# BGU-CS-VIL/DPMMSubClusters.jl

Measured on NVIDIA B200. Metric: gibbs_iters_per_sec, higher is better.
Workload: dtype f32

## Files before the change

dpmmsubclusters.jl_b200/_lib.py:

```python
from __future__ import annotations

import ctypes as C
import os

_HERE = os.path.dirname(os.path.abspath(__file__))
LIB_PATH = os.environ.get("DPMM_LIB_PATH") or os.path.join(_HERE, "libdpmm_b200.so")

OK, EINVAL, ECUDA, ESTATE, ELIMIT, ENCCL = 0, -1, -2, -3, -4, -5
PRIOR_NIW, PRIOR_MULTINOMIAL = 0, 1
SAMPLER_INVERSE_CDF, SAMPLER_GUMBEL = 0, 1

_p = C.c_void_p
_i32, _i64, _u64 = C.c_int32, C.c_int64, C.c_uint64
_f32p, _f64p, _i64p, _u8p = (C.POINTER(C.c_float), C.POINTER(C.c_double), C.POINTER(C.c_int64),
                             C.POINTER(C.c_uint8))

SIGNATURES = {
    "dpmm_create": (C.c_int, [C.POINTER(_p), _f32p, _i64, _i32, _i32, _i32, _u64, _i64]),
    "dpmm_destroy": (C.c_int, [_p]),
    "dpmm_last_error": (C.c_char_p, [_p]),
    "dpmm_set_stream": (C.c_int, [_p, _p]),
    "dpmm_sync": (C.c_int, [_p]),
    "dpmm_limits": (C.c_int, [C.POINTER(_i32)]),
    "dpmm_init_labels": (C.c_int, [_p, _i32, _i32]),
    "dpmm_randomize_sublabels": (C.c_int, [_p, _i64p, _i32]),
    "dpmm_get_labels": (C.c_int, [_p, _i64p]),
    "dpmm_get_sublabels": (C.c_int, [_p, _i64p]),
    "dpmm_set_labels": (C.c_int, [_p, _i64p]),
    "dpmm_set_sublabels": (C.c_int, [_p, _i64p]),
    "dpmm_set_params_niw": (C.c_int, [_p, _i32, _f32p, _f32p, _f32p, _f32p, _f32p]),
    "dpmm_set_params_multinomial": (C.c_int, [_p, _i32, _f32p, _f32p, _f32p]),
    "dpmm_set_sampler": (C.c_int, [_p, _i32]),
    "dpmm_sample_labels": (C.c_int, [_p, _i32]),
    "dpmm_sample_sublabels": (C.c_int, [_p]),
    "dpmm_suff_stats": (C.c_int, [_p, _i64p, _i32, _i64p, _f64p, _f64p]),
    "dpmm_num_clusters": (C.c_int, [_p]),
    "dpmm_set_hyper_niw": (C.c_int, [_p, C.c_double, _f64p, C.c_double, _f64p, C.c_double]),
    "dpmm_set_hyper_multinomial": (C.c_int, [_p, _f32p, C.c_double]),
    "dpmm_posterior_step": (C.c_int, [_p, _i64p, _i32, _i32, _u8p, _i32, _i64p, _f64p, _f64p]),
    "dpmm_sample_params": (C.c_int, [_p, _i32, _i32, _i32]),
    "dpmm_params_merge": (C.c_int, [_p, _i64, _i64]),
    "dpmm_get_params_niw": (C.c_int, [_p, _i32, _f32p, _f64p, _f32p, _f32p, _f32p]),
    "dpmm_get_params_multinomial": (C.c_int, [_p, _i32, _f32p, _f32p, _f32p]),
    "dpmm_predict_niw": (C.c_int, [_p, _i32, _f32p, _f32p, _f32p, _f32p, _i64p, _f32p]),
    "dpmm_predict_multinomial": (C.c_int, [_p, _i32, _f64p, _f32p, _i64p, _f32p]),
    "dpmm_apply_split": (C.c_int, [_p, _i64p, _i64p, _i32]),
    "dpmm_apply_merge": (C.c_int, [_p, _i64p, _i64p, _i32]),
    "dpmm_remove_empty": (C.c_int, [_p, _i64p, _i32]),
    "dpmm_smart_project": (C.c_int, [_p, _i64, _f64p, _f64p, _f64p, _i64p]),
    "dpmm_smart_kmeans_iter": (C.c_int, [_p, C.c_double, C.c_double, _f64p]),
    "dpmm_smart_set_sublabels": (C.c_int, [_p, _i64]),
    "dpmm_nccl_unique_id": (C.c_int, [_p]),
    "dpmm_comm_init": (C.c_int, [_p, _p, _i32, _i32]),
    "dpmm_set_uniforms": (C.c_int, [_p, _f64p, _f64p, _u8p]),
    "dpmm_debug_loglik": (C.c_int, [_p, _i32, _f32p]),
    "dpmm_debug_tc_stats": (C.c_int, [_p, _i64p]),
    "dpmm_debug_fused_stats": (C.c_int, [_p, _i64p]),
    "dpmm_timing_enable": (C.c_int, [_p, _i32]),
    "dpmm_timing_kinds": (C.c_int, []),
    "dpmm_timing_name": (C.c_char_p, [_i32]),
    "dpmm_timing_read": (C.c_int, [_p, _f64p, _i64p, _i32]),
    "dpmm_launch_count": (_i64, [_p]),
}

_lib = None


class DpmmError(RuntimeError):
    def __init__(self, code, msg):
        super().__init__(f"libdpmm_b200 error {code}: {msg}")
        self.code = code


def load():
    global _lib
    if _lib is not None:
        return _lib
    if not os.path.exists(LIB_PATH):
        raise FileNotFoundError(
            f"{LIB_PATH} is missing: build it with `python -c 'import __graft_entry__ as g; g.build()'` "
            "(nvcc, sm_100a). This package has no CPU fallback.")
    lib = C.CDLL(LIB_PATH)
    for name, (res, args) in SIGNATURES.items():
        fn = getattr(lib, name)
        fn.restype = res
        fn.argtypes = args
    _lib = lib
    return lib


def check(rc, ctx=None):
    if rc != 0:
        msg = load().dpmm_last_error(ctx)
        raise DpmmError(rc, msg.decode() if msg else "?")
```

dpmmsubclusters.jl_b200/csrc/common.cuh:

```cuda
#pragma once
#include <cuda_runtime.h>
#include <cstdint>
#include <math_constants.h>

#include "philox.cuh"

#define DPMM_MAX_K 1024
#define DPMM_MNM_MAX_D 16384

typedef unsigned long long f32x2_t;
__device__ __forceinline__ f32x2_t f2_pack(float lo, float hi) {
  f32x2_t r;
  asm("mov.b64 %0, {%1, %2};" : "=l"(r) : "f"(lo), "f"(hi));
  return r;
}
__device__ __forceinline__ void f2_unpack(f32x2_t v, float& lo, float& hi) {
  asm("mov.b64 {%0, %1}, %2;" : "=f"(lo), "=f"(hi) : "l"(v));
}
__device__ __forceinline__ f32x2_t f2_fma(f32x2_t a, f32x2_t b, f32x2_t c) {
  f32x2_t d;
  asm("fma.rn.f32x2 %0, %1, %2, %3;" : "=l"(d) : "l"(a), "l"(b), "l"(c));
  return d;
}

// ... 106 lines not shown
    const int k = __ffsll((long long)m) - 1;
    const float e = rs[k * stride];
    const bool zero = (e < 1.17549435e-38f) && s_regular;
    const float quo = __fdiv_rn(zero ? 1.f : e, s);
    cw = __fadd_rn(cw, zero ? 0.f : quo);
    rs[k * stride] = cw;
  }
  const double t = u * (double)cw;
  if (!(0.0 < t) && !(mask & 1ull)) return 0;
  for (uint64_t m = mask; m; m &= m - 1) {
    const int k = __ffsll((long long)m) - 1;
    if (k >= K - 1) break;
    if (!((double)rs[k * stride] < t)) return k;
  }
  return K - 1;
}

__device__ __forceinline__ int dpmm_draw_inverse_cdf_screened(float* rs, int stride, int K, double u) {
  if (K > 64) return dpmm_draw_inverse_cdf(rs, stride, K, u);
  float mx = -CUDART_INF_F;
  bool has_nan = false;
  for (int k = 0; k < K; ++k) {
    const float v = rs[k * stride];
    has_nan |= (v != v);
    mx = fmaxf(mx, v);
  }
  if (has_nan || !(mx > -CUDART_INF_F) || !(mx < CUDART_INF_F)) return dpmm_draw_inverse_cdf(rs, stride, K, u);
  const float thr = mx - 104.f;
  uint64_t mask = 0;
  for (int k = 0; k < K; ++k)
    if (rs[k * stride] >= thr) mask |= 1ull << k;
  if (2 * __popcll(mask) > K) return dpmm_draw_inverse_cdf(rs, stride, K, u);
  return dpmm_draw_inverse_cdf_masked(rs, stride, K, mask, u);
}

__device__ __forceinline__ int dpmm_draw_argmax(const float* rs, int stride, int K) {
  int best = 0;
  float bv = rs[0];
  if (bv != bv) return 0;
  for (int k = 1; k < K; ++k) {
    const float v = rs[k * stride];
    if (v != v) return k;
    if (v > bv) {
      bv = v;
      best = k;
    }
  }
  return best;
}

__device__ __forceinline__ int dpmm_draw_gumbel(const float* rs, int stride, int K, uint64_t seed,
                                               uint32_t call, uint64_t gidx) {
  int best = 0;
  float bv = -CUDART_INF_F;
  for (int k0 = 0; k0 < K; k0 += 4) {
    const Philox4 r = philox4x32_10((uint32_t)gidx, (uint32_t)(gidx >> 32), call,
                                    DPMM_STREAM_GUMBEL + 8u * (uint32_t)(k0 >> 2), (uint32_t)seed,
                                    (uint32_t)(seed >> 32));
    const uint32_t w[4] = {r.x, r.y, r.z, r.w};
#pragma unroll
    for (int j = 0; j < 4; ++j) {
      const int k = k0 + j;
      if (k < K) {
        float v = rs[k * stride];
        if (v != v) v = -CUDART_INF_F;
        const float uu = ((float)w[j] + 0.5f) * 2.3283064365386963e-10f;
        const float g = -__logf(-__logf(uu));
        const float t = v + g;
        if (t > bv || k == 0) {
          bv = t;
          best = k;
        }
      }
    }
  }
  return best;
}

__device__ __forceinline__ int dpmm_draw_two(float rl, float rr, double u) {
  float m[2] = {rl, rr};
  return dpmm_draw_inverse_cdf(m, 1, 2, u);
}

__device__ __forceinline__ double dpmm_uniform(const double* inj, int64_t local_i, uint64_t seed,
                                               uint32_t stream, uint32_t call, uint64_t gidx) {
  if (inj != nullptr) return inj[local_i];
  return philox_to_uniform(philox_draw(seed, stream, call, gidx));
}

__device__ __forceinline__ int dpmm_randbit(const uint8_t* inj, int64_t local_i, uint64_t seed,
                                            uint32_t call, uint64_t gidx) {
  if (inj != nullptr) return inj[local_i] & 1;
  return (int)(philox_draw(seed, DPMM_STREAM_RANDBITS, call, gidx).x & 1u);
}
```

dpmmsubclusters.jl_b200/csrc/ctx.cuh:

```cuda
#pragma once
#include "../../include/dpmm_b200.h"

#include <cuda.h>
#include <cuda_runtime.h>

#include <algorithm>
#include <cmath>
#include <cstdio>
#include <cstdlib>
#include <cstring>
#include <string>
#include <vector>

struct StatsItem;
struct SmartState;

enum TimingKind {
  TK_LABEL = 0,
  TK_SORT,
  TK_SUBLABEL,
  TK_STATS,
  TK_STATS_AUX,
  TK_RELABEL,
  TK_ALLREDUCE,
  TK_LABEL_OVF,
  TK_PARAMS,
  TK_COUNT
};
static const char* const kTimingNames[TK_COUNT] = {"label", "sort", "sublabel", "stats", "stats_aux", "relabel", "allreduce", "label_ovf", "params"};

struct TimedEvent {
  cudaEvent_t a, b;
  int kind;
};

struct UidBlob {
  char b[128];
};
struct NcclApi {
  void* handle = nullptr;
  int (*GetUniqueId)(void*) = nullptr;
  int (*CommInitRank)(void**, int, UidBlob, int) = nullptr;
  int (*AllReduce)(const void*, void*, size_t, int, int, void*, cudaStream_t) = nullptr;
  int (*AllGather)(const void*, void*, size_t, int, void*, cudaStream_t) = nullptr;
  int (*CommDestroy)(void*) = nullptr;
  const char* (*GetErrorString)(int) = nullptr;
};
struct dpmm_ctx {
  int device = 0;
  int sm_count = 148;
  int smem_optin = 0;
  int smem_per_sm = 0;
  cudaStream_t stream = nullptr;
  bool own_stream = true;
  cudaStream_t side = nullptr;
  cudaEvent_t ev_fork = nullptr, ev_join = nullptr;
  int64_t n = 0;
  int D = 0;
  int D_user = 0;
  int prior = 0;
  uint64_t seed = 0;
  int64_t goff = 0;
  uint32_t call = 0;
  int sampler = 0;
  std::string err;

  float* x = nullptr;
  int32_t* labels = nullptr;
  uint8_t* sub = nullptr;
  int32_t* perm = nullptr;
  int32_t* perm2 = nullptr;
  int64_t* wide = nullptr;
  int32_t* wide_status = nullptr;
  double* u_label = nullptr;
  double* u_sub = nullptr;
  uint8_t* r_bits = nullptr;

  int K = 0, Kcap = 0;
  int label_bound = 1;
  bool params_set = false;
  int rec_f = 0;
  float* raw_params = nullptr;
  float* recs = nullptr;
  float* cst = nullptr;
  float* logw = nullptr;
  float* loglr = nullptr;
  float* tc_w = nullptr;
  float* tc_b = nullptr;
  float* tc_mu = nullptr;
  float* tc_fro = nullptr;
  int32_t* tc_stats = nullptr;
  float* t2_piv = nullptr;
  float* t2_scr = nullptr;
  float* t2_u = nullptr;
  float* t2_bias = nullptr;
  float* t2_fro8 = nullptr;
  int32_t* t2_ctr = nullptr;
  int32_t* ctr_sets = nullptr;
  int ctr_cur = 0;
  bool ctr_clean = false;
  bool t2_ok = false;
  bool t2_params = false;
  int t2_KS = 0, t2_nch = 0;
  int32_t* t2_hstat = nullptr;
  cudaEvent_t t2_hstat_ev = nullptr;
  bool t2_hstat_pending = false;
  int t2_cooldown = 0;
  float* ss_w = nullptr;
  float* ss_b = nullptr;
  float* ss_c = nullptr;
  int32_t* lcount = nullptr;
  CUtensorMap tmap_x;
  float* mtc_w = nullptr;
  bool mtc_ok = false;
  bool mtc_params = false;
  bool tc_ok = false;
  bool tc_params = false;
  float* logp_t = nullptr;
  int KP = 0;
  int32_t* hist = nullptr;
  int32_t* seg_off = nullptr;
  int32_t* scat_cursor = nullptr;
  int32_t* lr_cursor = nullptr;
  int32_t* lut_l = nullptr;
  int32_t* lut_r = nullptr;
  uint8_t* rule = nullptr;
  uint8_t* wanted = nullptr;
  int32_t* idx_list = nullptr;
  int stats_rec = 0;
  double* acc = nullptr;
  float* centers = nullptr;
  double* outbuf = nullptr;
  StatsItem* items = nullptr;
  int64_t items_cap = 0;
  int32_t* item_ctr = nullptr;
  int chunk = 1024;

  void* hstage = nullptr;
  size_t hstage_bytes = 0;
  void* hup[2] = {nullptr, nullptr};
  size_t hup_bytes[2] = {0, 0};
  cudaEvent_t hup_ev[2] = {nullptr, nullptr};
  int hup_i = 0;

  bool hist_valid = false, sorted = false, partitioned = false;
  bool scan_valid = false;
  int64_t n_fused = 0, n_cached = 0, n_recompute = 0;
  bool acc_cleared = false;
  bool stats_cached = false;
  bool cursors_fresh = false;
  int64_t launches = 0;
  bool timing = false;
  std::vector<TimedEvent> tev;
  std::vector<cudaEvent_t> ev_pool;
  double t_ms[TK_COUNT] = {0};
  int64_t t_n[TK_COUNT] = {0};

  bool dev_params = false;
  double alpha = 0.0;
  double* hyper_d = nullptr;
  double* ptab = nullptr;
  double* ptab_alt = nullptr;
  double* post = nullptr;
  double* post_alt = nullptr;
  double* lfac = nullptr;
  double* pm_out = nullptr;
  uint8_t* splittable_d = nullptr;
  int32_t* newof_d = nullptr;
  float* w_out = nullptr;
  float* lr_out = nullptr;
  uint32_t pcall = 0;
  int Kcap_tab = 0;

  SmartState* smart = nullptr;

  NcclApi nccl;
  void* comm = nullptr;
  int world = 1, rank = 0;
  bool ipc_ok = false;
  uint8_t* ipc_local = nullptr;
  uint8_t* ipc_peer[16] = {nullptr};
  size_t ipc_cap = 0;
  uint32_t ipc_epoch = 0;
};

void dpmm_internal_smart_free(dpmm_ctx* ctx);
int dpmm_internal_ensure_sorted(dpmm_ctx* ctx);

inline thread_local std::string g_err;

inline int fail(dpmm_ctx* c, int code, const std::string& msg) {
  if (c) c->err = msg;
  g_err = msg;
  return code;
}
#define CK(call)                                                                                   \
  do {                                                                                             \
    cudaError_t e__ = (call);                                                                      \
    if (e__ != cudaSuccess)                                                                        \
      return fail(ctx, DPMM_ECUDA, std::string(#call) + ": " + cudaGetErrorString(e__));          \
  } while (0)
#define NEED(cond, code, msg) \
  do {                        \
// ... 99 lines not shown
```

dpmmsubclusters.jl_b200/csrc/dpmm_b200.cu:

```cuda

#include <dlfcn.h>

#include <algorithm>
#include <cmath>
#include <cstdio>
#include <cstring>
#include <string>
#include <vector>

#include "common.cuh"
#include "kernels_gauss.cuh"
#include "kernels_gauss_tc.cuh"
#include "kernels_gauss_tc2.cuh"
#include "kernels_ipc.cuh"
#include "kernels_mnm.cuh"
#include "kernels_mnm_tc.cuh"
#include "kernels_pack.cuh"
#include "kernels_params.cuh"
#include "kernels_params_mnm.cuh"
#include "kernels_sort.cuh"
#include "kernels_stats.cuh"
#include "kernels_stats_tc.cuh"
#include "kernels_stats_tc64.cuh"
#include "kernels_substats_tc.cuh"
// ... 8 lines not shown
  return gauss_col_off(D) + ((D + 3) & ~3);
}

template <typename T>
static cudaError_t dev_grow_keep(T** p, size_t old_count, size_t new_count) {
  T* q = nullptr;
  cudaError_t e = cudaMalloc((void**)&q, std::max<size_t>(new_count, 1) * sizeof(T));
  if (e != cudaSuccess) return e;
  e = cudaMemset(q, 0, std::max<size_t>(new_count, 1) * sizeof(T));
  if (e == cudaSuccess && *p && old_count) e = cudaMemcpy(q, *p, old_count * sizeof(T), cudaMemcpyDeviceToDevice);
  if (*p) cudaFree(*p);
  *p = q;
  return e;
}
static int post_doubles(const dpmm_ctx* c) {
  return c->prior == DPMM_PRIOR_NIW ? NIW_POST_DOUBLES(c->D) : MNM_POST_DOUBLES(c->D);
}
static int ensure_tables(dpmm_ctx* ctx, int cap) {
  if (cap <= ctx->Kcap_tab) return 0;
  CK(cudaStreamSynchronize(ctx->stream));
  const int D = ctx->D, old = ctx->Kcap_tab;
  const bool niw = ctx->prior == DPMM_PRIOR_NIW;
  const size_t rec3 = (size_t)3 * (niw ? 1 + D + D * D : 1 + D), post3 = (size_t)3 * post_doubles(ctx);
  CK(dev_grow_keep(&ctx->ptab, old * rec3, cap * rec3));
  CK(dev_grow_keep(&ctx->ptab_alt, 0, cap * rec3));
  CK(dev_grow_keep(&ctx->post, old * post3, cap * post3));
  CK(dev_grow_keep(&ctx->post_alt, 0, cap * post3));
  if (niw) CK(dev_grow_keep(&ctx->lfac, (size_t)3 * old * D * D, (size_t)3 * cap * D * D));
  CK(dev_grow_keep(&ctx->pm_out, 0, (size_t)cap * 6 + (size_t)cap * cap + 2));
  CK(dev_grow_keep(&ctx->splittable_d, 0, (size_t)cap));
  CK(dev_grow_keep(&ctx->newof_d, 0, (size_t)cap));
  CK(dev_grow_keep(&ctx->w_out, (size_t)old, (size_t)cap));
  CK(dev_grow_keep(&ctx->lr_out, (size_t)2 * old, (size_t)2 * cap));
  ctx->Kcap_tab = cap;
  return 0;
}

static int ensure_k(dpmm_ctx* ctx, int K) {
  if (K <= ctx->Kcap) return 0;
  int cap = std::max(K, std::max(8, ctx->Kcap * 2));
  cap = std::min(cap, DPMM_MAX_K);
  if (K > cap) return fail(ctx, DPMM_ELIMIT, "K exceeds DPMM_MAX_K");
  CK(cudaStreamSynchronize(ctx->stream));
  const int D = ctx->D;
  ctx->rec_f = nrec_floats(ctx);
  ctx->stats_rec = (ctx->prior == DPMM_PRIOR_NIW) ? 1 + D + D * D : 1 + D;
  CK(dev_realloc(&ctx->recs, (size_t)3 * cap * ctx->rec_f));
  if (ctx->prior == DPMM_PRIOR_NIW) CK(dev_realloc(&ctx->raw_params, (size_t)3 * cap * (D + D * D + 1)));
  CK(dev_realloc(&ctx->cst, (size_t)3 * cap));
  CK(dev_realloc(&ctx->logw, (size_t)cap));
  CK(dev_realloc(&ctx->loglr, (size_t)2 * cap));
  if (ctx->prior == DPMM_PRIOR_MULTINOMIAL) CK(dev_realloc(&ctx->logp_t, (size_t)D * (cap + MNM_KT)));
  if (ctx->mtc_ok) {
    CK(dev_realloc(&ctx->mtc_w, (size_t)3 * ((D + 31) / 32) * MTC_N * 32));
    ctx->mtc_params = false;
  }
  if (ctx->tc_ok || ctx->t2_ok) {
    CK(dev_realloc(&ctx->tc_b, (size_t)cap * D));
    CK(dev_realloc(&ctx->tc_mu, (size_t)cap * D));
    CK(dev_realloc(&ctx->tc_fro, (size_t)cap));
    ctx->tc_params = ctx->t2_params = false;
  }
  if (ctx->t2_ok) {
    const int capt = std::min(cap, T2_MAX_K);
    CK(dev_realloc(&ctx->t2_piv, (size_t)capt * D * D));
    CK(dev_realloc(&ctx->t2_u, (size_t)capt * D * D));
    CK(dev_realloc(&ctx->t2_scr, (size_t)gauss_tc2_nch(D, capt) * (D / 8) * 1024));
    CK(dev_realloc(&ctx->t2_bias, (size_t)capt * (gauss_tc2_nch(D, capt) * 512 + 32)));
    CK(dev_realloc(&ctx->t2_fro8, (size_t)capt));
  }
  if (ctx->tc_ok) {
    const int capc = std::min(cap, TC_MAX_K);
    CK(dev_realloc(&ctx->tc_w, (size_t)((capc + TC_NCL - 1) / TC_NCL) * TC_NCL * TC_D * TC_D));
    CK(dev_realloc(&ctx->ss_w, (size_t)cap * 2 * SS_D * SS_D));
    CK(dev_realloc(&ctx->ss_b, (size_t)cap * 2 * SS_D));
    CK(dev_realloc(&ctx->ss_c, (size_t)cap * SS_D));
    CK(dev_realloc(&ctx->lcount, (size_t)cap));
  }
  if (ctx->prior == DPMM_PRIOR_NIW && D == L64_D) {
    CK(dev_realloc(&ctx->ss_w, (size_t)cap * 2 * D * D));
    CK(dev_realloc(&ctx->ss_b, (size_t)cap * 2 * D));
    CK(dev_realloc(&ctx->ss_c, (size_t)cap * D));
  }
  CK(dev_realloc(&ctx->hist, (size_t)cap));
  CK(dev_realloc(&ctx->seg_off, (size_t)cap + 1));
  CK(dev_realloc(&ctx->scat_cursor, (size_t)cap));
  CK(dev_realloc(&ctx->lr_cursor, (size_t)2 * cap));
  CK(dev_realloc(&ctx->lut_l, (size_t)cap));
  CK(dev_realloc(&ctx->lut_r, (size_t)cap));
  CK(dev_realloc(&ctx->rule, (size_t)cap));
  CK(dev_realloc(&ctx->wanted, (size_t)cap));
  CK(dev_realloc(&ctx->idx_list, (size_t)cap));
  CK(dev_realloc(&ctx->acc, (size_t)2 * cap * ctx->stats_rec));
  CK(dev_realloc(&ctx->centers, (size_t)2 * cap * ctx->D));
  CK(dev_realloc(&ctx->outbuf, (size_t)3 * cap * ctx->stats_rec + 1));
  ctx->items_cap = ctx->n / ctx->chunk + 2 * (int64_t)cap + 2;
  CK(dev_realloc(&ctx->items, (size_t)ctx->items_cap));
  ctx->Kcap = cap;
  ctx->hist_valid = ctx->scan_valid = ctx->sorted = ctx->partitioned = ctx->stats_cached = false;
  ctx->params_set = false;
  ctx->acc_cleared = ctx->cursors_fresh = false;
  if (ctx->dev_params) {
    int rc = ensure_tables(ctx, cap);
    if (rc) return rc;
  }
  return 0;
}

#define DPMM_NIW_DIMS(X) X(1) X(2) X(3) X(4) X(5) X(6) X(7) X(8) X(12) X(16) X(24) X(32) X(48) X(64)

static bool niw_dim_supported(int D) {
  switch (D) {
#define X(d) case d:
    DPMM_NIW_DIMS(X)
#undef X
    return true;
    default:
      return false;
  }
}

#define DECL_SET(n)                                                                              \
  int niw_set_label_##n(dpmm_ctx*, const GaussLabelArgs&, int, int*);                            \
  int niw_set_sublabel_##n(dpmm_ctx*, const SubLabelArgs&, bool, int, int*);                     \
  int niw_set_stats_##n(dpmm_ctx*, const StatsArgs&, int, int*);
DECL_SET(0) DECL_SET(1) DECL_SET(2) DECL_SET(3) DECL_SET(4) DECL_SET(5)
#undef DECL_SET

int niw_launch_label(dpmm_ctx* ctx, const GaussLabelArgs& a) {
  int rc = DPMM_ELIMIT;
  const int D = ctx->D;
  if (niw_set_label_0(ctx, a, D, &rc) && niw_set_label_1(ctx, a, D, &rc) && niw_set_label_2(ctx, a, D, &rc) &&
      niw_set_label_3(ctx, a, D, &rc) && niw_set_label_4(ctx, a, D, &rc) && niw_set_label_5(ctx, a, D, &rc))
    return fail(ctx, DPMM_ELIMIT, "NIW: no kernel instantiated for this D");
  return rc;
}
int niw_launch_sublabel(dpmm_ctx* ctx, const SubLabelArgs& a, bool sample) {
  int rc = DPMM_ELIMIT;
  const int D = ctx->D;
  if (niw_set_sublabel_0(ctx, a, sample, D, &rc) && niw_set_sublabel_1(ctx, a, sample, D, &rc) &&
      niw_set_sublabel_2(ctx, a, sample, D, &rc) && niw_set_sublabel_3(ctx, a, sample, D, &rc) &&
      niw_set_sublabel_4(ctx, a, sample, D, &rc) && niw_set_sublabel_5(ctx, a, sample, D, &rc))
    return fail(ctx, DPMM_ELIMIT, "NIW: no kernel instantiated for this D");
  return rc;
}
int niw_launch_stats(dpmm_ctx* ctx, const StatsArgs& a) {
  int rc = DPMM_ELIMIT;
  const int D = ctx->D;
  if (niw_set_stats_0(ctx, a, D, &rc) && niw_set_stats_1(ctx, a, D, &rc) && niw_set_stats_2(ctx, a, D, &rc) &&
      niw_set_stats_3(ctx, a, D, &rc) && niw_set_stats_4(ctx, a, D, &rc) && niw_set_stats_5(ctx, a, D, &rc))
    return fail(ctx, DPMM_ELIMIT, "NIW: no kernel instantiated for this D");
  return rc;
}

extern "C" const char* dpmm_last_error(const dpmm_ctx* ctx) { return ctx ? ctx->err.c_str() : g_err.c_str(); }

extern "C" int dpmm_limits(int32_t* out3) {
  if (!out3) return DPMM_EINVAL;
  out3[0] = 64;
  out3[1] = DPMM_MNM_MAX_D;
  out3[2] = DPMM_MAX_K;
  return 0;
}

extern "C" int dpmm_create(dpmm_ctx** out, const float* x, int64_t n_local, int32_t d, int32_t prior_kind,
                           int32_t device, uint64_t seed, int64_t global_offset) {
  dpmm_ctx* ctx = nullptr;
// ... 6 lines not shown
  if (prior_kind == DPMM_PRIOR_NIW) {
    NEED(d <= 64, DPMM_ELIMIT, "NIW: D must be <= 64");
    while (!niw_dim_supported(dpad)) ++dpad;
  } else
    NEED(d <= DPMM_MNM_MAX_D, DPMM_ELIMIT, "multinomial: D must be <= 16384");
  int ndev = 0;
  if (cudaGetDeviceCount(&ndev) != cudaSuccess || ndev == 0)
    return fail(nullptr, DPMM_ECUDA, "no CUDA device: libdpmm_b200 has no CPU fallback");
  NEED(device >= 0 && device < ndev, DPMM_EINVAL, "bad device ordinal");
  ctx = new dpmm_ctx();
  ctx->device = device;
  ctx->n = n_local;
  ctx->D = dpad;
  ctx->D_user = d;
  ctx->prior = prior_kind;
  ctx->seed = seed;
  ctx->goff = global_offset;
  auto bail = [&](int code) {
    g_err = ctx->err;
    dpmm_destroy(ctx);
    return code;
  };
#define CKC(call)                                                                        \
  do {                                                                                   \
    cudaError_t e__ = (call);                                                            \
    if (e__ != cudaSuccess) {                                                            \
      ctx->err = std::string(#call) + ": " + cudaGetErrorString(e__);                    \
      return bail(DPMM_ECUDA);                                                           \
    }                                                                                    \
  } while (0)
  CKC(cudaSetDevice(device));
  cudaDeviceProp prop;
  CKC(cudaGetDeviceProperties(&prop, device));
  if (prop.major < 10) {
    ctx->err = "device is not sm_100-class (Blackwell); this library ships sm_100a code only";
    return bail(DPMM_ECUDA);
  }
  ctx->sm_count = prop.multiProcessorCount;
  ctx->smem_optin = (int)prop.sharedMemPerBlockOptin;
  ctx->smem_per_sm = (int)prop.sharedMemPerMultiprocessor;
  CKC(cudaStreamCreateWithFlags(&ctx->stream, cudaStreamNonBlocking));
  CKC(cudaMalloc((void**)&ctx->x, (size_t)n_local * dpad * sizeof(float)));
  CKC(cudaMalloc((void**)&ctx->labels, (size_t)n_local * sizeof(int32_t)));
  CKC(cudaMalloc((void**)&ctx->sub, (size_t)n_local));
  CKC(cudaMalloc((void**)&ctx->perm, (size_t)n_local * sizeof(int32_t)));
  CKC(cudaMalloc((void**)&ctx->perm2, (size_t)n_local * sizeof(int32_t)));
  CKC(cudaMalloc((void**)&ctx->item_ctr, 2 * sizeof(int32_t)));
  if (dpad == d) {
    CKC(cudaMemcpyAsync(ctx->x, x, (size_t)n_local * d * sizeof(float), cudaMemcpyHostToDevice, ctx->stream));
  } else {
    float* raw = nullptr;
    CKC(cudaMalloc((void**)&raw, (size_t)n_local * d * sizeof(float)));
    cudaError_t e1 = cudaMemcpyAsync(raw, x, (size_t)n_local * d * sizeof(float), cudaMemcpyHostToDevice, ctx->stream);
    if (e1 == cudaSuccess) {
      pad_points_kernel<<<(unsigned)prop.multiProcessorCount * 8, 256, 0, ctx->stream>>>(raw, n_local, d, dpad, ctx->x);
      e1 = cudaGetLastError();
    }
    if (e1 == cudaSuccess) e1 = cudaStreamSynchronize(ctx->stream);
    cudaFree(raw);
    CKC(e1);
  }
  CKC(cudaMemsetAsync(ctx->labels, 0, (size_t)n_local * sizeof(int32_t), ctx->stream));
  CKC(cudaMemsetAsync(ctx->sub, 0, (size_t)n_local, ctx->stream));
  CKC(cudaStreamSynchronize(ctx->stream));
  if (prior_kind == DPMM_PRIOR_NIW && dpad == TC_D && n_local >= TC_TILE) {
    typedef CUresult (*EncodeFn)(CUtensorMap*, CUtensorMapDataType, cuuint32_t, void*, const cuuint64_t*, const cuuint64_t*,
                                 const cuuint32_t*, const cuuint32_t*, CUtensorMapInterleave, CUtensorMapSwizzle,
                                 CUtensorMapL2promotion, CUtensorMapFloatOOBfill);
    void* fn = nullptr;
    cudaDriverEntryPointQueryResult qres;
    if (cudaGetDriverEntryPoint("cuTensorMapEncodeTiled", &fn, cudaEnableDefault, &qres) == cudaSuccess && fn != nullptr &&
        qres == cudaDriverEntryPointSuccess) {
      const cuuint64_t gdim[2] = {(cuuint64_t)TC_D, (cuuint64_t)n_local};
      const cuuint64_t gstr[1] = {(cuuint64_t)TC_D * 4};
      const cuuint32_t box[2] = {TC_D, TC_TILE};
      const cuuint32_t estr[2] = {1, 1};
      const CUresult r = ((EncodeFn)fn)(&ctx->tmap_x, CU_TENSOR_MAP_DATA_TYPE_FLOAT32, 2, ctx->x, gdim, gstr, box, estr,
                                        CU_TENSOR_MAP_INTERLEAVE_NONE, CU_TENSOR_MAP_SWIZZLE_128B,
                                        CU_TENSOR_MAP_L2_PROMOTION_L2_128B, CU_TENSOR_MAP_FLOAT_OOB_FILL_NONE);
      ctx->tc_ok = (r == CUDA_SUCCESS);
    }
  }
  if (ctx->tc_ok || (prior_kind == DPMM_PRIOR_NIW && (dpad == 32 || dpad == 64) && n_local >= T2_TILE)) {
    CKC(cudaMalloc((void**)&ctx->ctr_sets, 8 * sizeof(int32_t)));
    CKC(cudaMemset(ctx->ctr_sets, 0, 8 * sizeof(int32_t)));
    ctx->tc_stats = ctx->ctr_sets;
    ctx->t2_ctr = ctx->ctr_sets + 2;
  }
  if (prior_kind == DPMM_PRIOR_NIW && (dpad == 32 || dpad == 64) && n_local >= T2_TILE) ctx->t2_ok = true;
  if (prior_kind == DPMM_PRIOR_MULTINOMIAL && d % 4 == 0 && d <= MTC_MAX_D && n_local >= MTC_TILE) {
    bool exact = false;
    {
      int32_t* flag = nullptr;
      int32_t hflag = 1;
      if (cudaMalloc((void**)&flag, 4) == cudaSuccess) {
        cudaMemsetAsync(flag, 0, 4, ctx->stream);
        tf32_exact_scan_kernel<<<(unsigned)ctx->sm_count * 16, 256, 0, ctx->stream>>>(ctx->x, (int64_t)n_local * d, flag);
        if (cudaMemcpyAsync(&hflag, flag, 4, cudaMemcpyDeviceToHost, ctx->stream) == cudaSuccess &&
            cudaStreamSynchronize(ctx->stream) == cudaSuccess)
          exact = hflag == 0;
        cudaFree(flag);
      }
    }
    typedef CUresult (*EncodeFn)(CUtensorMap*, CUtensorMapDataType, cuuint32_t, void*, const cuuint64_t*, const cuuint64_t*,
                                 const cuuint32_t*, const cuuint32_t*, CUtensorMapInterleave, CUtensorMapSwizzle,
                                 CUtensorMapL2promotion, CUtensorMapFloatOOBfill);
    void* fn = nullptr;
    cudaDriverEntryPointQueryResult qres;
    if (exact && cudaGetDriverEntryPoint("cuTensorMapEncodeTiled", &fn, cudaEnableDefault, &qres) == cudaSuccess &&
        fn != nullptr && qres == cudaDriverEntryPointSuccess) {
      const cuuint64_t gdim[2] = {(cuuint64_t)d, (cuuint64_t)n_local};
      const cuuint64_t gstr[1] = {(cuuint64_t)d * 4};
      const cuuint32_t box[2] = {32, MTC_TILE};
      const cuuint32_t estr[2] = {1, 1};
      const CUresult r = ((EncodeFn)fn)(&ctx->tmap_x, CU_TENSOR_MAP_DATA_TYPE_FLOAT32, 2, ctx->x, gdim, gstr, box, estr,
                                        CU_TENSOR_MAP_INTERLEAVE_NONE, CU_TENSOR_MAP_SWIZZLE_128B,
                                        CU_TENSOR_MAP_L2_PROMOTION_L2_128B, CU_TENSOR_MAP_FLOAT_OOB_FILL_NONE);
      ctx->mtc_ok = (r == CUDA_SUCCESS);
    }
  }
#undef CKC
  ctx->chunk = prior_kind == DPMM_PRIOR_NIW ? 1024 : 256;
  *out = ctx;
  return 0;
}

extern "C" int dpmm_destroy(dpmm_ctx* ctx) {
  if (!ctx) return 0;
  cudaSetDevice(ctx->device);
  if (ctx->stream) cudaStreamSynchronize(ctx->stream);
  if (env_int("DPMM_VERBOSE", 0))
    fprintf(stderr, "[dpmm] fused sub-label+statistics launches %lld, statistics served from them %lld, exact recomputations %lld\n",
            (long long)ctx->n_fused, (long long)ctx->n_cached, (long long)ctx->n_recompute);
  for (int p = 0; p < IPC_MAX_WORLD; ++p)
    if (ctx->ipc_peer[p]) cudaIpcCloseMemHandle(ctx->ipc_peer[p]);
  if (ctx->ipc_local) cudaFree(ctx->ipc_local);
  dpmm_internal_smart_free(ctx);
  if (ctx->side) {
    cudaStreamSynchronize(ctx->side);
    cudaStreamDestroy(ctx->side);
    cudaEventDestroy(ctx->ev_fork);
    cudaEventDestroy(ctx->ev_join);
  }
  if (ctx->comm && ctx->nccl.CommDestroy) ctx->nccl.CommDestroy(ctx->comm);
  for (auto& t : ctx->tev) {
    cudaEventDestroy(t.a);
    cudaEventDestroy(t.b);
  }
  for (auto e : ctx->ev_pool) cudaEventDestroy(e);
  void* ptrs[] = {ctx->x, ctx->labels, ctx->sub, ctx->perm, ctx->perm2, ctx->u_label, ctx->u_sub, ctx->r_bits,
                  ctx->raw_params, ctx->recs, ctx->cst, ctx->logw, ctx->loglr, ctx->logp_t, ctx->t2_piv, ctx->t2_scr, ctx->t2_u, ctx->t2_bias, ctx->t2_fro8, ctx->ctr_sets, ctx->tc_w, ctx->tc_b, ctx->tc_mu, ctx->tc_fro, ctx->ss_w, ctx->ss_b, ctx->ss_c, ctx->lcount, ctx->mtc_w, ctx->hist, ctx->seg_off,
                  ctx->scat_cursor, ctx->lr_cursor, ctx->lut_l, ctx->lut_r, ctx->rule, ctx->wanted,
                  ctx->idx_list, ctx->acc, ctx->centers, ctx->outbuf, ctx->items, ctx->item_ctr, ctx->hyper_d, ctx->ptab,
                  ctx->ptab_alt, ctx->post, ctx->post_alt, ctx->lfac, ctx->pm_out, ctx->splittable_d, ctx->newof_d,
                  ctx->w_out, ctx->lr_out, ctx->wide, ctx->wide_status};
  for (void* p : ptrs)
    if (p) cudaFree(p);
  if (ctx->hstage) cudaFreeHost(ctx->hstage);
  if (ctx->t2_hstat) cudaFreeHost(ctx->t2_hstat);
  if (ctx->t2_hstat_ev) cudaEventDestroy(ctx->t2_hstat_ev);
  for (int i = 0; i < 2; ++i) {
    if (ctx->hup[i]) cudaFreeHost(ctx->hup[i]);
    if (ctx->hup_ev[i]) cudaEventDestroy(ctx->hup_ev[i]);
  }
  if (ctx->own_stream && ctx->stream) cudaStreamDestroy(ctx->stream);
  delete ctx;
  return 0;
}

extern "C" int dpmm_set_stream(dpmm_ctx* ctx, void* cuda_stream) {
  NEED(ctx, DPMM_EINVAL, "ctx is NULL");
  CK(cudaSetDevice(ctx->device));
  CK(cudaStreamSynchronize(ctx->stream));
  if (ctx->own_stream && ctx->stream) cudaStreamDestroy(ctx->stream);
  ctx->stream = (cudaStream_t)cuda_stream;
  ctx->own_stream = false;
  return 0;
}

extern "C" int dpmm_sync(dpmm_ctx* ctx) {
  NEED(ctx, DPMM_EINVAL, "ctx is NULL");
  CK(cudaSetDevice(ctx->device));
  CK(cudaStreamSynchronize(ctx->stream));
  return 0;
}

extern "C" int dpmm_set_sampler(dpmm_ctx* ctx, int32_t sampler) {
  NEED(ctx, DPMM_EINVAL, "ctx is NULL");
  NEED(sampler == DPMM_SAMPLER_INVERSE_CDF || sampler == DPMM_SAMPLER_GUMBEL, DPMM_EINVAL, "unknown sampler");
  ctx->sampler = sampler;
  return 0;
}

static int run_relabel(dpmm_ctx* ctx, const std::vector<int32_t>& ll, const std::vector<int32_t>& lr,
                       const std::vector<uint8_t>& rule, bool uses_rng) {
  const int K = (int)ll.size();
  int rc = ensure_k(ctx, K);
  if (rc) return rc;
  const size_t b4 = (size_t)K * 4;
  void* hs = nullptr;
  const int slot = upload_acquire(ctx, 2 * b4 + K, &hs);
  if (slot < 0) return slot;
  char* h = (char*)hs;
  memcpy(h, ll.data(), b4);
  memcpy(h + b4, lr.data(), b4);
  memcpy(h + 2 * b4, rule.data(), K);
  CK(cudaMemcpyAsync(ctx->lut_l, h, b4, cudaMemcpyHostToDevice, ctx->stream));
  CK(cudaMemcpyAsync(ctx->lut_r, h + b4, b4, cudaMemcpyHostToDevice, ctx->stream));
  CK(cudaMemcpyAsync(ctx->rule, h + 2 * b4, K, cudaMemcpyHostToDevice, ctx->stream));
  rc = upload_release(ctx, slot);
  if (rc) return rc;
  if (uses_rng) ctx->call += 1;
  {
    KernelTimer kt(ctx, TK_RELABEL);
    const int T = 256;
    const unsigned grid = (unsigned)std::min<int64_t>((ctx->n + T - 1) / T, (int64_t)ctx->sm_count * 16);
    relabel_kernel<<<grid, T, 0, ctx->stream>>>(ctx->labels, ctx->sub, ctx->n, K, ctx->lut_l, ctx->lut_r, ctx->rule,
                                                ctx->r_bits, ctx->seed, ctx->call, ctx->goff);
    CK(cudaGetLastError());
  }
  return 0;
}

extern "C" int dpmm_init_labels(dpmm_ctx* ctx, int32_t init_clusters, int32_t outlier) {
  NEED(ctx, DPMM_EINVAL, "ctx is NULL");
  NEED(init_clusters >= 1 && init_clusters + (outlier ? 1 : 0) <= DPMM_MAX_K, DPMM_EINVAL, "bad init_clusters");
  CK(cudaSetDevice(ctx->device));
  ctx->label_bound = init_clusters + (outlier ? 1 : 0);
  {
    int rc = ensure_k(ctx, ctx->label_bound);
    if (rc) return rc;
  }
  ctx->call += 1;
  {
// ... 301 lines not shown
  const size_t raw_floats = nrec * D + nrec * D * D + nrec;
  const size_t bytes = (raw_floats + K + 2 * K) * sizeof(float);
  void* hs = nullptr;
  const int slot = upload_acquire(ctx, bytes, &hs);
  if (slot < 0) return slot;
  float* h_mu = (float*)hs;
  float* h_inv = h_mu + nrec * D;
  float* h_ld = h_inv + nrec * D * D;
  float* h_logw = h_ld + nrec;
  float* h_loglr = h_logw + K;
  if (Du == D) {
    memcpy(h_mu, mu, nrec * D * 4);
    memcpy(h_inv, inv_sigma, nrec * D * D * 4);
  } else {
    memset(h_mu, 0, nrec * D * 4);
    memset(h_inv, 0, nrec * D * D * 4);
    for (size_t t = 0; t < nrec; ++t) {
      memcpy(h_mu + t * D, mu + t * Du, (size_t)Du * 4);
      for (int i = 0; i < Du; ++i) memcpy(h_inv + (t * D + i) * D, inv_sigma + (t * Du + i) * Du, (size_t)Du * 4);
      for (int i = Du; i < D; ++i) h_inv[(t * D + i) * D + i] = 1.f;
    }
  }
  memcpy(h_ld, logdet, nrec * 4);
  common_weights(ctx, K, weights, lr_weights, h_logw, h_loglr);
  CK(cudaMemcpyAsync(ctx->raw_params, h_mu, raw_floats * 4, cudaMemcpyHostToDevice, ctx->stream));
  CK(cudaMemcpyAsync(ctx->logw, h_logw, (size_t)K * 4, cudaMemcpyHostToDevice, ctx->stream));
  CK(cudaMemcpyAsync(ctx->loglr, h_loglr, (size_t)2 * K * 4, cudaMemcpyHostToDevice, ctx->stream));
  rc = upload_release(ctx, slot);
  if (rc) return rc;
  rc = niw_pack_launch(ctx, K, nullptr);
  if (rc) return rc;
  return 0;
}

static int mnm_pack_launch(dpmm_ctx* ctx, int K) {
  const int D = ctx->D;
  const int KP = (K + MNM_KT - 1) / MNM_KT * MNM_KT;
  const bool mtc = ctx->mtc_ok && K <= MTC_MAX_K;
  MnmPackArgs pa{};
  pa.D = D; pa.K = K; pa.KP = KP; pa.logp = ctx->recs; pa.logp_t = ctx->logp_t; pa.mtc_w = mtc ? ctx->mtc_w : nullptr;
  const int64_t ne = std::max<int64_t>((int64_t)D * KP, mtc ? (int64_t)((D + 31) / 32) * MTC_N * 32 : 0);
  {
    KernelTimer kt(ctx, TK_PARAMS);
    mnm_pack_kernel<<<(unsigned)std::min<int64_t>((ne + 255) / 256, (int64_t)ctx->sm_count * 4), 256, 0, ctx->stream>>>(pa);
    CK(cudaGetLastError());
  }
  ctx->mtc_params = mtc;
  ctx->K = K;
  ctx->KP = KP;
  ctx->params_set = true;
  return 0;
}

extern "C" int dpmm_set_params_multinomial(dpmm_ctx* ctx, int32_t K, const float* log_p, const float* weights,
                                           const float* lr_weights) {
  NEED(ctx, DPMM_EINVAL, "ctx is NULL");
  NEED(ctx->prior == DPMM_PRIOR_MULTINOMIAL, DPMM_ESTATE, "context was created with the NIW prior");
  NEED(K >= 1 && K <= DPMM_MAX_K, DPMM_ELIMIT, "K out of range");
  NEED(log_p && weights && lr_weights, DPMM_EINVAL, "NULL parameter array");
  CK(cudaSetDevice(ctx->device));
  int rc = ensure_k(ctx, K);
  if (rc) return rc;
  const int D = ctx->D;
  const size_t nrec = (size_t)3 * K;
  const size_t bytes = (nrec * D + K + 2 * K) * sizeof(float);
  void* hs = nullptr;
  const int slot = upload_acquire(ctx, bytes, &hs);
  if (slot < 0) return slot;
  float* h_recs = (float*)hs;
  float* h_logw = h_recs + nrec * D;
  float* h_loglr = h_logw + K;
  memcpy(h_recs, log_p, nrec * D * 4);
  common_weights(ctx, K, weights, lr_weights, h_logw, h_loglr);
  CK(cudaMemcpyAsync(ctx->recs, h_recs, nrec * D * 4, cudaMemcpyHostToDevice, ctx->stream));
  CK(cudaMemcpyAsync(ctx->logw, h_logw, (size_t)K * 4, cudaMemcpyHostToDevice, ctx->stream));
  CK(cudaMemcpyAsync(ctx->loglr, h_loglr, (size_t)2 * K * 4, cudaMemcpyHostToDevice, ctx->stream));
  rc = upload_release(ctx, slot);
  if (rc) return rc;
  return mnm_pack_launch(ctx, K);
}

static int ensure_sorted(dpmm_ctx* ctx);

template <int D>
static int launch_label_tc2(dpmm_ctx* ctx, int final_iter, int nkeys) {
  const int K = ctx->K;
  GaussTc2Args a{};
  a.x = ctx->x; a.n = ctx->n; a.K = K; a.KS = ctx->t2_KS; a.nch = ctx->t2_nch; a.n0 = gauss_tc2_n0(D);
  a.perm = ctx->perm; a.seg_off = ctx->seg_off; a.nkeys = nkeys; a.wpiv = ctx->t2_piv; a.wscr = ctx->t2_scr;
  a.wbias = ctx->t2_bias; a.fro8 = ctx->t2_fro8;
  a.urows = ctx->t2_u; a.mu = ctx->tc_mu; a.cst = ctx->cst; a.logw = ctx->logw; a.fro = ctx->tc_fro;
  ctx->ctr_cur ^= 1;
  ctx->tc_stats = ctx->ctr_sets + 4 * ctx->ctr_cur;
  ctx->t2_ctr = ctx->tc_stats + 2;
  a.labels = ctx->labels; a.hist = ctx->hist; a.ovf_list = ctx->perm2; a.ovf_count = ctx->t2_ctr;
  a.u_inj = ctx->u_label; a.seed = ctx->seed; a.call = ctx->call; a.goff = ctx->goff; a.final_iter = final_iter;
  a.stats = ctx->tc_stats;
  const size_t sm = GaussTc2Smem(D, K, a.KS, a.nch, nkeys).total;
  CK(cudaFuncSetAttribute(gauss_label_tc2_kernel<D>, cudaFuncAttributeMaxDynamicSharedMemorySize, (int)sm));
  if (!ctx->ctr_clean) CK(cudaMemsetAsync(ctx->ctr_sets, 0, 8 * sizeof(int32_t), ctx->stream));
  const int64_t grid = std::min<int64_t>((ctx->n + T2_TILE - 1) / T2_TILE, (int64_t)ctx->sm_count);
  {
    KernelTimer kt(ctx, TK_LABEL);
    gauss_label_tc2_kernel<D><<<(unsigned)grid, T2_THREADS(D), sm, ctx->stream>>>(a);
    CK(cudaGetLastError());
  }
  GaussListArgs l{};
  l.x = ctx->x; l.K = K; l.list = ctx->perm2; l.count = ctx->t2_ctr; l.urows = ctx->t2_u; l.mu = ctx->tc_mu;
  l.cst = ctx->cst; l.logw = ctx->logw; l.labels = ctx->labels; l.hist = ctx->hist; l.u_inj = ctx->u_label;
  l.seed = ctx->seed; l.call = ctx->call; l.goff = ctx->goff; l.final_iter = final_iter; l.stats = a.stats;
  l.zero_next = ctx->ctr_sets + 4 * (ctx->ctr_cur ^ 1);
  ctx->ctr_clean = true;
  l.ticket = ctx->tc_stats + 3; l.scan_k = K; l.seg_off = ctx->seg_off; l.scat_cursor = ctx->scat_cursor; l.lr_cursor = ctx->lr_cursor;
  const size_t lsm = (size_t)8 * K * 4;
  if (lsm > 48 * 1024) CK(cudaFuncSetAttribute(gauss_label_list_kernel<D>, cudaFuncAttributeMaxDynamicSharedMemorySize, (int)lsm));
  {
    KernelTimer kt(ctx, TK_LABEL_OVF);
    gauss_label_list_kernel<D><<<(unsigned)ctx->sm_count * 2, 256, lsm, ctx->stream>>>(l);
    CK(cudaGetLastError());
  }
  if (ctx->t2_hstat == nullptr) {
    CK(cudaMallocHost((void**)&ctx->t2_hstat, 4 * sizeof(int32_t)));
    CK(cudaEventCreateWithFlags(&ctx->t2_hstat_ev, cudaEventDisableTiming));
  }
  CK(cudaMemcpyAsync(ctx->t2_hstat, ctx->tc_stats, 12, cudaMemcpyDeviceToHost, ctx->stream));
  CK(cudaEventRecord(ctx->t2_hstat_ev, ctx->stream));
  ctx->t2_hstat_pending = true;
  return 0;
}

template <int TP>
static int launch_mnm_label_stream(dpmm_ctx* ctx, MnmLabelArgs& a) {
  const size_t sm = MnmStreamCfg<TP>::smem_bytes(a.K);
  NEED(sm <= (size_t)ctx->smem_optin, DPMM_ELIMIT, "internal: multinomial streaming label kernel does not fit shared memory");
  a.ntiles = (a.n + TP - 1) / TP;
  CK(cudaFuncSetAttribute(mnm_label_stream_kernel<TP>, cudaFuncAttributeMaxDynamicSharedMemorySize, (int)sm));
  int occ = 1;
  CK(cudaOccupancyMaxActiveBlocksPerMultiprocessor(&occ, mnm_label_stream_kernel<TP>, 256, sm));
  occ = std::max(occ, 1);
  const int64_t grid = std::min<int64_t>(a.ntiles, (int64_t)ctx->sm_count * occ);
  KernelTimer kt(ctx, TK_LABEL);
  mnm_label_stream_kernel<TP><<<(unsigned)grid, 256, sm, ctx->stream>>>(a);
  CK(cudaGetLastError());
  return 0;
}

static int run_sample_labels(dpmm_ctx* ctx, int final_iter, float* dump) {
  NEED(ctx->params_set, DPMM_ESTATE, "set_params must precede sample_labels");
  const int K = ctx->K;
  ctx->call += 1;
  bool use_t2 = ctx->prior == DPMM_PRIOR_NIW && ctx->t2_params && dump == nullptr &&
                ctx->sampler == DPMM_SAMPLER_INVERSE_CDF && env_int("DPMM_LABEL_TC", 2) == 2;
  if (use_t2 && env_int("DPMM_LABEL_ADAPT", 1) != 0) {
    if (ctx->t2_hstat_pending && cudaEventQuery(ctx->t2_hstat_ev) == cudaSuccess) {
      ctx->t2_hstat_pending = false;
      const double pts = std::max(1, ctx->t2_hstat[0]);
      const double evals = (double)ctx->t2_hstat[1] / pts;
      if (evals > 0.03 * K + 0.05) ctx->t2_cooldown = 8;
    }
    if (ctx->t2_cooldown > 0) {
      --ctx->t2_cooldown;
      use_t2 = false;
    }
  }
  int nkeys = 0;
  if (use_t2) {
    nkeys = keff(ctx);
    use_t2 = GaussTc2Smem(ctx->D, K, ctx->t2_KS, ctx->t2_nch, nkeys).total <= (size_t)ctx->smem_optin;
  }
  if (use_t2) {
    int rc = ensure_sorted(ctx);
    if (rc) return rc;
  }
  CK(cudaMemsetAsync(ctx->hist, 0, (size_t)K * 4, ctx->stream));
  if (use_t2) {
    int rc = ctx->D == 32 ? launch_label_tc2<32>(ctx, final_iter, nkeys) : launch_label_tc2<64>(ctx, final_iter, nkeys);
    if (rc) return rc;
  } else if (ctx->prior == DPMM_PRIOR_NIW && ctx->tc_params && dump == nullptr && ctx->sampler == DPMM_SAMPLER_INVERSE_CDF &&
      env_int("DPMM_LABEL_TC", 2) != 0) {
    GaussTcArgs a{};
    a.n = ctx->n; a.K = K; a.wmat = ctx->tc_w; a.bvec = ctx->tc_b; a.mu = ctx->tc_mu; a.cst = ctx->cst; a.logw = ctx->logw;
    a.fro = ctx->tc_fro; a.labels = ctx->labels; a.hist = ctx->hist; a.u_inj = ctx->u_label; a.seed = ctx->seed;
    a.call = ctx->call; a.goff = ctx->goff; a.final_iter = final_iter; a.ntiles = (ctx->n + TC_TILE - 1) / TC_TILE;
    a.stats = env_int("DPMM_TC_STATS", 0) ? ctx->tc_stats : nullptr;
    const size_t sm = GaussTcSmem(K).total;
    NEED(sm <= (size_t)ctx->smem_optin, DPMM_ELIMIT, "internal: tensor-core label kernel does not fit shared memory");
    CK(cudaFuncSetAttribute(gauss_label_tc_kernel, cudaFuncAttributeMaxDynamicSharedMemorySize, (int)sm));
    const int64_t grid = std::min<int64_t>((a.ntiles + 1) / 2, (int64_t)ctx->sm_count);
    if (a.stats) {
      CK(cudaMemsetAsync(ctx->tc_stats, 0, 8, ctx->stream));
      ctx->ctr_clean = false;
    }
    KernelTimer kt(ctx, TK_LABEL);
    gauss_label_tc_kernel<<<(unsigned)grid, TC_THREADS, sm, ctx->stream>>>(ctx->tmap_x, a);
    CK(cudaGetLastError());
  } else if (ctx->prior == DPMM_PRIOR_NIW) {
    GaussLabelArgs a{};
    a.x = ctx->x; a.n = ctx->n; a.K = K; a.recs = ctx->recs; a.cst = ctx->cst; a.logw = ctx->logw;
    a.labels = ctx->labels; a.hist = ctx->hist; a.u_inj = ctx->u_label; a.seed = ctx->seed; a.call = ctx->call;
    a.goff = ctx->goff; a.final_iter = final_iter; a.sampler = ctx->sampler; a.dump = dump;
    int rc = niw_launch_label(ctx, a);
    if (rc) return rc;
  } else if (ctx->mtc_params && dump == nullptr && env_int("DPMM_LABEL_TC", 1) != 0) {
    MnmTcArgs a{};
    a.n = ctx->n; a.D = ctx->D; a.K = K; a.NP = (ctx->D + 31) / 32; a.wsplit = ctx->mtc_w; a.logw = ctx->logw;
    a.labels = ctx->labels; a.hist = ctx->hist; a.u_inj = ctx->u_label; a.seed = ctx->seed; a.call = ctx->call;
    a.goff = ctx->goff; a.final_iter = final_iter; a.sampler = ctx->sampler; a.ntiles = (ctx->n + MTC_TILE - 1) / MTC_TILE;
    a.NG = MnmTcSmem(K, a.NP, MTC_NG).total <= (size_t)ctx->smem_optin ? MTC_NG : 2;
    const size_t sm = MnmTcSmem(K, a.NP, a.NG).total;
    NEED(sm <= (size_t)ctx->smem_optin, DPMM_ELIMIT, "internal: multinomial tensor-core kernel does not fit shared memory");
    CK(cudaFuncSetAttribute(mnm_label_tc_kernel, cudaFuncAttributeMaxDynamicSharedMemorySize, (int)sm));
    const int64_t grid = std::min<int64_t>(a.ntiles, (int64_t)ctx->sm_count);
    KernelTimer kt(ctx, TK_LABEL);
    mnm_label_tc_kernel<<<(unsigned)grid, MTC_THREADS(a.NG), sm, ctx->stream>>>(ctx->tmap_x, a);
    CK(cudaGetLastError());
  } else {
    MnmLabelArgs a{};
    a.x = ctx->x; a.n = ctx->n; a.D = ctx->D; a.DS = ctx->D | 1; a.K = K; a.KP = ctx->KP; a.logp_t = ctx->logp_t;
    a.logw = ctx->logw; a.labels = ctx->labels; a.hist = ctx->hist; a.u_inj = ctx->u_label; a.seed = ctx->seed;
    a.call = ctx->call; a.goff = ctx->goff; a.final_iter = final_iter; a.sampler = ctx->sampler; a.dump = dump;
    int T = 128;
    auto bytes = [&](int T_) { return ((size_t)a.D * a.KP + (size_t)T_ * a.DS + (size_t)K * T_) * 4 + (size_t)K * 4; };
    while (T > 32 && bytes(T) > (size_t)ctx->smem_optin) T /= 2;
    if (bytes(T) <= (size_t)ctx->smem_optin) {
      a.ntiles = (a.n + T - 1) / T;
      const size_t sm = bytes(T);
      CK(cudaFuncSetAttribute(mnm_label_kernel, cudaFuncAttributeMaxDynamicSharedMemorySize, (int)sm));
      int occ = 1;
      CK(cudaOccupancyMaxActiveBlocksPerMultiprocessor(&occ, mnm_label_kernel, T, sm));
      occ = std::max(occ, 1);
      const int64_t grid = std::min<int64_t>(a.ntiles, (int64_t)ctx->sm_count * occ);
      KernelTimer kt(ctx, TK_LABEL);
      mnm_label_kernel<<<(unsigned)grid, T, sm, ctx->stream>>>(a);
      CK(cudaGetLastError());
    } else {
      int rc = MnmStreamCfg<128>::smem_bytes(K) <= (size_t)ctx->smem_optin ? launch_mnm_label_stream<128>(ctx, a)
             : MnmStreamCfg<64>::smem_bytes(K) <= (size_t)ctx->smem_optin  ? launch_mnm_label_stream<64>(ctx, a)
                                                                            : launch_mnm_label_stream<32>(ctx, a);
      if (rc) return rc;
    }
  }
  ctx->hist_valid = true;
  ctx->scan_valid = use_t2;
  ctx->sorted = false;
  ctx->partitioned = ctx->stats_cached = false;
  ctx->label_bound = K;
  return 0;
}

static int ensure_sorted(dpmm_ctx* ctx) {
  if (ctx->sorted) return 0;
  const int K = keff(ctx);
  {
    int rc = ensure_k(ctx, K);
    if (rc) return rc;
  }
  KernelTimer kt(ctx, TK_SORT, 1 + (ctx->hist_valid ? 0 : 1) + (ctx->hist_valid && ctx->scan_valid ? 0 : 1));
  if (!ctx->hist_valid) {
    CK(cudaMemsetAsync(ctx->hist, 0, (size_t)K * 4, ctx->stream));
    const int T = 256;
    const unsigned grid = (unsigned)std::min<int64_t>((ctx->n + T - 1) / T, (int64_t)ctx->sm_count * 8);
    label_hist_kernel<<<grid, T, (size_t)K * 4, ctx->stream>>>(ctx->labels, ctx->n, K, ctx->hist);
    CK(cudaGetLastError());
    ctx->hist_valid = true;
  }
  if (!(ctx->hist_valid && ctx->scan_valid)) {
    label_scan_kernel<<<1, 1024, 0, ctx->stream>>>(ctx->hist, K, ctx->seg_off, ctx->scat_cursor, ctx->lr_cursor);
    CK(cudaGetLastError());
  }
  ctx->scan_valid = false;
  {
    const int T = 256;
    const unsigned grid = (unsigned)((ctx->n + (int64_t)T * SCATTER_PPT - 1) / ((int64_t)T * SCATTER_PPT));
    const bool pre = ctx->prior == DPMM_PRIOR_NIW && ctx->D == SS_D && ctx->tc_ok && ctx->lcount != nullptr;
    label_scatter_kernel<<<grid, T, (size_t)K * 8, ctx->stream>>>(ctx->labels, ctx->n, K, ctx->scat_cursor, ctx->perm,
                                                                  pre ? ctx->acc : nullptr, pre ? (int64_t)2 * K * ctx->stats_rec : 0,
                                                                  pre ? ctx->lcount : nullptr, pre ? K : 0);
    CK(cudaGetLastError());
    ctx->acc_cleared = pre;
  }
  ctx->sorted = true;
  ctx->partitioned = ctx->stats_cached = false;
  ctx->cursors_fresh = true;
  return 0;
}

int dpmm_internal_ensure_sorted(dpmm_ctx* ctx) { return ensure_sorted(ctx); }

static int run_sublabels(dpmm_ctx* ctx, bool sample, float* dump) {
  int rc = ensure_sorted(ctx);
  if (rc) return rc;
  if (!ctx->cursors_fresh) {
    KernelTimer kt(ctx, TK_SORT);
    label_scan_kernel<<<1, 1024, 0, ctx->stream>>>(ctx->hist, keff(ctx), ctx->seg_off, ctx->scat_cursor,
                                                   ctx->lr_cursor);
    CK(cudaGetLastError());
  }
  SubLabelArgs a{};
  a.x = ctx->x; a.n = ctx->n; a.K = ctx->K; a.recs = ctx->recs; a.cst = ctx->cst; a.loglr = ctx->loglr;
  a.labels = ctx->labels; a.sub = ctx->sub; a.perm = ctx->perm; a.perm2 = ctx->perm2; a.cursor = ctx->lr_cursor;
  a.seg_off = ctx->seg_off;
  a.u_inj = ctx->u_sub; a.seed = ctx->seed; a.call = ctx->call; a.goff = ctx->goff; a.dump = dump; a.D = ctx->D;
  if (sample && ctx->prior == DPMM_PRIOR_NIW && ctx->D == SS_D && ctx->tc_ok && env_int("DPMM_SUBSTATS_TC", 1) != 0 &&
      SubStatsSmem(ctx->K).total <= (size_t)ctx->smem_optin && keff(ctx) == ctx->K) {
    const int K = ctx->K, recs = ctx->stats_rec;
    if (!ctx->acc_cleared) {
      CK(cudaMemsetAsync(ctx->acc, 0, (size_t)2 * K * recs * 8, ctx->stream));
      CK(cudaMemsetAsync(ctx->lcount, 0, (size_t)K * 4, ctx->stream));
    }
    ctx->acc_cleared = false;
    SubStatsArgs f{};
    f.x = ctx->x; f.n = ctx->n; f.K = K; f.perm = ctx->perm; f.seg_off = ctx->seg_off; f.w = ctx->ss_w; f.bias = ctx->ss_b;
    f.cen = ctx->ss_c; f.cst = ctx->cst; f.loglr = ctx->loglr; f.sub = ctx->sub; f.acc = ctx->acc; f.rec = recs;
    f.lcount = ctx->lcount; f.centers = ctx->centers; f.u_inj = ctx->u_sub; f.seed = ctx->seed; f.call = ctx->call;
    f.goff = ctx->goff; f.dump = dump;
    const size_t smem = SubStatsSmem(K).total;
    CK(cudaFuncSetAttribute(niw_substats_tc_kernel, cudaFuncAttributeMaxDynamicSharedMemorySize, (int)smem));
    {
      KernelTimer kt(ctx, TK_SUBLABEL);
      niw_substats_tc_kernel<<<ctx->sm_count, SS_THREADS, smem, ctx->stream>>>(f);
      CK(cudaGetLastError());
    }
    ctx->partitioned = false;
    ctx->stats_cached = true;
    ++ctx->n_fused;
    return 0;
  }
  if (sample && ctx->prior == DPMM_PRIOR_NIW && ctx->D == L64_D && ctx->ss_w != nullptr && env_int("DPMM_SUBLABEL_TC64", 1) != 0 &&
      SubLabel64Smem(ctx->K).total <= (size_t)ctx->smem_optin && keff(ctx) == ctx->K && ctx->n >= L64_TILE) {
    SubLabel64Args f{};
    f.x = ctx->x; f.n = ctx->n; f.K = ctx->K; f.perm = ctx->perm; f.seg_off = ctx->seg_off; f.w = ctx->ss_w; f.bias = ctx->ss_b;
    f.cen = ctx->ss_c; f.cst = ctx->cst; f.loglr = ctx->loglr; f.sub = ctx->sub; f.u_inj = ctx->u_sub; f.seed = ctx->seed;
    f.call = ctx->call; f.goff = ctx->goff; f.dump = dump; f.perm2 = ctx->perm2; f.cursor = ctx->lr_cursor;
    const size_t smem = SubLabel64Smem(ctx->K).total;
    CK(cudaFuncSetAttribute(niw_sublabel_tc64_kernel, cudaFuncAttributeMaxDynamicSharedMemorySize, (int)smem));
    KernelTimer kt(ctx, TK_SUBLABEL);
    niw_sublabel_tc64_kernel<<<ctx->sm_count, L64_THREADS, smem, ctx->stream>>>(f);
    CK(cudaGetLastError());
    ctx->partitioned = true;
    ctx->cursors_fresh = false;
    ctx->stats_cached = false;
    return 0;
  }
  if (ctx->prior == DPMM_PRIOR_NIW) {
    rc = niw_launch_sublabel(ctx, a, sample);
    if (rc) return rc;
  } else {
    const int T = 128;
    const unsigned grid = (unsigned)((a.n + T - 1) / T);
    KernelTimer kt(ctx, TK_SUBLABEL);
    if (sample && ctx->D <= 128)
      mnm_sublabel2_kernel<<<grid, T, 0, ctx->stream>>>(a);
    else if (sample && ctx->D > 1024)
      mnm_sublabel_staged_kernel<<<grid, MNM_SLS_T, 0, ctx->stream>>>(a);
    else if (sample)
      mnm_sublabel_kernel<true><<<grid, T, 0, ctx->stream>>>(a);
    else
      mnm_sublabel_kernel<false><<<grid, T, 0, ctx->stream>>>(a);
    CK(cudaGetLastError());
  }
  ctx->partitioned = true;
  ctx->cursors_fresh = false;
  return 0;
}

extern "C" int dpmm_sample_labels(dpmm_ctx* ctx, int32_t final_iter) {
  NEED(ctx, DPMM_EINVAL, "ctx is NULL");
  CK(cudaSetDevice(ctx->device));
  return run_sample_labels(ctx, final_iter, nullptr);
}

extern "C" int dpmm_sample_sublabels(dpmm_ctx* ctx) {
  NEED(ctx, DPMM_EINVAL, "ctx is NULL");
  CK(cudaSetDevice(ctx->device));
  NEED(ctx->params_set, DPMM_ESTATE, "set_params must precede sample_sublabels");
  NEED(ctx->label_bound <= ctx->K, DPMM_ESTATE, "labels refer to clusters beyond the K of set_params");
  ctx->call += 1;
  return run_sublabels(ctx, true, nullptr);
}

struct StatsCall {
  int m = 0;
  bool all = false, cached = false;
};
static int stats_compute(dpmm_ctx* ctx, const int64_t* indices, int32_t n_indices, StatsCall* sc) {
  const int K = keff(ctx);
  int rc = ensure_k(ctx, K);
  if (rc) return rc;
  const int D = ctx->D, rec = ctx->stats_rec;
  std::vector<int32_t> idx;
  if (indices == nullptr) {
    idx.resize(K);
    for (int k = 0; k < K; ++k) idx[k] = k;
  } else {
    NEED(n_indices >= 0, DPMM_EINVAL, "n_indices < 0");
    idx.resize(n_indices);
    for (int i = 0; i < n_indices; ++i) {
      NEED(indices[i] >= 1 && indices[i] <= K, DPMM_EINVAL, "cluster index out of range [1, K]");
      idx[i] = (int32_t)indices[i] - 1;
    }
  }
  const int m = (int)idx.size();
  sc->m = m;
  if (m == 0) return 0;
// ... 8 lines not shown
  sc->cached = cached;
  rc = ensure_stage(ctx, std::max<size_t>((size_t)m * 4 + K, ((size_t)m * 3 * rec + 1) * 8));
  if (rc) return rc;
  if (!all) {
    CK(cudaStreamSynchronize(ctx->stream));
    int32_t* h_idx = (int32_t*)ctx->hstage;
    uint8_t* h_w = (uint8_t*)(h_idx + m);
    memcpy(h_idx, idx.data(), (size_t)m * 4);
    CK(cudaMemcpyAsync(ctx->idx_list, h_idx, (size_t)m * 4, cudaMemcpyHostToDevice, ctx->stream));
    memset(h_w, 0, K);
    for (int v : idx) h_w[v] = 1;
    CK(cudaMemcpyAsync(ctx->wanted, h_w, K, cudaMemcpyHostToDevice, ctx->stream));
  }
  const bool stats_tc = !cached && ctx->prior == DPMM_PRIOR_NIW && D == STC_D && all && ctx->tc_ok &&
                        env_int("DPMM_STATS_TC", 1) != 0 && StatsTcSmem(K).total <= (size_t)ctx->smem_optin;
  const bool stats_tc64 = !cached && ctx->prior == DPMM_PRIOR_NIW && D == S64_D && all && env_int("DPMM_STATS_TC", 1) != 0 &&
                          StatsTc64Smem(K).total <= (size_t)ctx->smem_optin;
  if (cached) {
  } else if (!stats_tc && !stats_tc64) {
    KernelTimer kt(ctx, TK_STATS_AUX);
    stats_worklist_kernel<<<1, 256, (size_t)2 * K * 4, ctx->stream>>>(ctx->seg_off, ctx->lr_cursor,
                                                                      all ? nullptr : ctx->wanted, K, ctx->chunk,
                                                                      ctx->items, ctx->item_ctr, ctx->item_ctr + 1);
    CK(cudaGetLastError());
  }
  if (!cached) {
    CK(cudaMemsetAsync(ctx->acc, 0, (size_t)2 * K * rec * 8, ctx->stream));
    ctx->acc_cleared = false;
  }
  StatsArgs sa{};
  sa.x = ctx->x; sa.D = D; sa.perm2 = ctx->perm2; sa.items = ctx->items; sa.n_items = ctx->item_ctr;
  sa.next_item = ctx->item_ctr + 1; sa.acc = ctx->acc; sa.rec = rec;
  if (cached) {
  } else if (stats_tc) {
    StatsTcArgs ta{};
    ta.x = ctx->x; ta.perm2 = ctx->perm2; ta.seg_off = ctx->seg_off; ta.lr_cursor = ctx->lr_cursor; ta.K = K;
    ta.acc = ctx->acc; ta.rec = rec; ta.centers = ctx->centers;
    {
      KernelTimer kt(ctx, TK_STATS_AUX);
      stats_centers_kernel<<<2 * K, 256, 0, ctx->stream>>>(ctx->x, ctx->perm2, ctx->seg_off, ctx->lr_cursor, ctx->centers);
      CK(cudaGetLastError());
    }
    const size_t smem = StatsTcSmem(K).total;
    CK(cudaFuncSetAttribute(niw_stats_tc_kernel, cudaFuncAttributeMaxDynamicSharedMemorySize, (int)smem));
    CK(cudaFuncSetAttribute(niw_stats_tc_kernel, cudaFuncAttributePreferredSharedMemoryCarveout, cudaSharedmemCarveoutMaxShared));
    const int occ = 2 * (smem + 1024) <= (size_t)ctx->smem_per_sm ? 2 : 1;
    KernelTimer kt(ctx, TK_STATS);
    niw_stats_tc_kernel<<<ctx->sm_count * occ, STC_THREADS, smem, ctx->stream>>>(ta);
    CK(cudaGetLastError());
  } else if (stats_tc64) {
    StatsTcArgs ta{};
    ta.x = ctx->x; ta.perm2 = ctx->perm2; ta.seg_off = ctx->seg_off; ta.lr_cursor = ctx->lr_cursor; ta.K = K;
    ta.acc = ctx->acc; ta.rec = rec; ta.centers = ctx->centers;
    {
      KernelTimer kt(ctx, TK_STATS_AUX);
      stats_centers64_kernel<<<2 * K, 512, 0, ctx->stream>>>(ctx->x, ctx->perm2, ctx->seg_off, ctx->lr_cursor, ctx->centers);
      CK(cudaGetLastError());
    }
    const size_t smem = StatsTc64Smem(K).total;
    CK(cudaFuncSetAttribute(niw_stats_tc64_kernel, cudaFuncAttributeMaxDynamicSharedMemorySize, (int)smem));
    KernelTimer kt(ctx, TK_STATS);
    niw_stats_tc64_kernel<<<ctx->sm_count, S64_THREADS, smem, ctx->stream>>>(ta);
    CK(cudaGetLastError());
  } else if (ctx->prior == DPMM_PRIOR_NIW) {
    rc = niw_launch_stats(ctx, sa);
    if (rc) return rc;
  } else {
    const auto kern = D > 32 * MNM_STATS_NREG ? mnm_stats_kernel<true> : mnm_stats_kernel<false>;
    int occ = 1;
    CK(cudaOccupancyMaxActiveBlocksPerMultiprocessor(&occ, kern, 256, 0));
    occ = std::max(occ, 1);
    KernelTimer kt(ctx, TK_STATS);
    kern<<<ctx->sm_count * occ, 256, 0, ctx->stream>>>(sa);
    CK(cudaGetLastError());
  }
  const size_t nred = (size_t)m * 3 * rec + 1;
  const bool use_ipc = ctx->comm != nullptr && ctx->ipc_ok && nred <= ctx->ipc_cap;
  const uint32_t epoch = use_ipc ? ++ctx->ipc_epoch : 0;
  double* fin = use_ipc ? reinterpret_cast<double*>(ctx->ipc_local + IPC_FLAG_BYTES) + (size_t)(epoch & 1) * ctx->ipc_cap : ctx->outbuf;
  {
    KernelTimer kt(ctx, TK_STATS_AUX);
    const int T = 256;
    dim3 grid((unsigned)std::min((rec + T - 1) / T, 64), (unsigned)m);
    CK(cudaMemsetAsync(fin + (size_t)m * 3 * rec, 0, 8, ctx->stream));
    stats_finalize_kernel<<<grid, T, 0, ctx->stream>>>(ctx->acc, ctx->seg_off, ctx->lr_cursor, all ? nullptr : ctx->idx_list, m, D, rec,
                                                       ctx->prior == DPMM_PRIOR_NIW ? 1 : 0, fin,
                                                       (stats_tc || stats_tc64 || cached) ? ctx->centers : nullptr,
                                                       cached ? ctx->lcount : nullptr,
                                                       cached ? fin + (size_t)m * 3 * rec : nullptr);
    CK(cudaGetLastError());
  }
  if (use_ipc) {
    IpcReduceArgs ia{};
    ia.world = ctx->world; ia.rank = ctx->rank; ia.epoch = epoch; ia.n = nred; ia.out = ctx->outbuf;
    ia.my_flags = reinterpret_cast<const uint32_t*>(ctx->ipc_local);
    for (int r = 0; r < ctx->world; ++r) {
      uint8_t* base = r == ctx->rank ? ctx->ipc_local : ctx->ipc_peer[r];
      ia.src[r] = reinterpret_cast<const double*>(base + IPC_FLAG_BYTES) + (size_t)(epoch & 1) * ctx->ipc_cap;
      ia.peer_flags[r] = reinterpret_cast<uint32_t*>(base);
    }
    KernelTimer kt(ctx, TK_ALLREDUCE);
    const unsigned grid = (unsigned)std::min<size_t>((nred / 2 + 255) / 256, (size_t)ctx->sm_count * 4);
    ipc_allreduce_kernel<<<grid, 256, 0, ctx->stream>>>(ia);
    CK(cudaGetLastError());
  } else if (ctx->comm != nullptr) {
    KernelTimer kt(ctx, TK_ALLREDUCE);
    const int r = ctx->nccl.AllReduce(ctx->outbuf, ctx->outbuf, (size_t)m * 3 * rec + 1,  8,  0,
                                      ctx->comm, ctx->stream);
    if (r != 0) return fail(ctx, DPMM_ENCCL, std::string("ncclAllReduce: ") + ctx->nccl.GetErrorString(r));
  }
  return 0;
}

extern "C" int dpmm_suff_stats(dpmm_ctx* ctx, const int64_t* indices, int32_t n_indices, int64_t* counts,
                               double* sum_x, double* sum_xx) {
  NEED(ctx, DPMM_EINVAL, "ctx is NULL");
  CK(cudaSetDevice(ctx->device));
  if (indices == nullptr && n_indices > 0)
    NEED(n_indices == keff(ctx), DPMM_EINVAL,
         "indices == NULL means every cluster: n_indices must be 0 or the number of label values in use "
         "(max of the K of set_params and the largest label); the output arrays hold that many rows");
  StatsCall sc;
  int rc = stats_compute(ctx, indices, n_indices, &sc);
  if (rc) return rc;
  const int m = sc.m, D = ctx->D, rec = ctx->stats_rec;
  const bool cached = sc.cached;
  if (m == 0) return 0;
  if (counts == nullptr && sum_x == nullptr && sum_xx == nullptr) return 0;
  double* h = (double*)ctx->hstage;
  CK(cudaMemcpyAsync(h, ctx->outbuf, ((size_t)m * 3 * rec + (cached ? 1 : 0)) * 8, cudaMemcpyDeviceToHost, ctx->stream));
  CK(cudaStreamSynchronize(ctx->stream));
  if (cached && h[(size_t)m * 3 * rec] != 0.0) {
    ctx->stats_cached = false;
    ++ctx->n_recompute;
    return dpmm_suff_stats(ctx, indices, n_indices, counts, sum_x, sum_xx);
  }
  if (cached) ++ctx->n_cached;
  for (int a = 0; a < m; ++a)
    for (int s = 0; s < 3; ++s) {
      const double* r = h + ((size_t)a * 3 + s) * rec;
      if (counts) counts[a * 3 + s] = (int64_t)llround(r[0]);
      const int Du = ctx->D_user;
      if (sum_x) memcpy(sum_x + ((size_t)a * 3 + s) * Du, r + 1, (size_t)Du * 8);
      if (sum_xx && ctx->prior == DPMM_PRIOR_NIW)
        for (int i = 0; i < Du; ++i)
          memcpy(sum_xx + (((size_t)a * 3 + s) * Du + i) * Du, r + 1 + D + (size_t)i * D, (size_t)Du * 8);
    }
  return 0;
}


extern "C" int dpmm_num_clusters(const dpmm_ctx* ctx) { return ctx ? keff(ctx) : 0; }

extern "C" int dpmm_set_hyper_niw(dpmm_ctx* ctx, double kappa, const double* m, double nu, const double* psi, double alpha) {
  NEED(ctx && m && psi, DPMM_EINVAL, "NULL argument");
  NEED(ctx->prior == DPMM_PRIOR_NIW, DPMM_ESTATE, "context was created with the multinomial prior");
  NEED(ctx->D == ctx->D_user, DPMM_ELIMIT,
       "the device-side parameter step needs an instantiated feature dimension (1-8, 12, 16, 24, 32, 48, 64); "
       "sample the parameters on the host (dpmm_set_params_niw) for other D");
  NEED(kappa > 0 && nu > ctx->D - 1 && alpha > 0, DPMM_EINVAL, "need kappa > 0, nu > D - 1, alpha > 0");
  CK(cudaSetDevice(ctx->device));
  const int D = ctx->D;
  std::vector<double> h(NIW_HYPER_DOUBLES(D));
  std::vector<double> A((size_t)D * D);
  for (int i = 0; i < D; ++i)
    for (int j = 0; j < D; ++j) A[(size_t)i * D + j] = 0.5 * (psi[(size_t)i * D + j] + psi[(size_t)j * D + i]);
  double logdet = 0.0;
  for (int j = 0; j < D; ++j) {
    double d = A[(size_t)j * D + j];
    for (int k = 0; k < j; ++k) d -= A[(size_t)j * D + k] * A[(size_t)j * D + k];
    NEED(d > 0 && std::isfinite(d), DPMM_EINVAL, "psi must be positive definite");
    const double l = std::sqrt(d);
    A[(size_t)j * D + j] = l;
// ... 372 lines not shown
                                ctx->stream>>>(dscore, n, K, dlab, probs != nullptr);
    CKP(cudaGetLastError());
  }
  std::vector<int32_t> h((size_t)n);
  CKP(cudaMemcpyAsync(h.data(), dlab, (size_t)n * 4, cudaMemcpyDeviceToHost, ctx->stream));
  if (probs) CKP(cudaMemcpyAsync(probs, dscore, (size_t)n * K * 4, cudaMemcpyDeviceToHost, ctx->stream));
  CKP(cudaStreamSynchronize(ctx->stream));
#undef CKP
  for (int64_t i = 0; i < n; ++i) labels[i] = (int64_t)h[i] + 1;
  cleanup();
  return 0;
}

extern "C" int dpmm_debug_loglik(dpmm_ctx* ctx, int32_t which, float* out) {
  NEED(ctx && out, DPMM_EINVAL, "NULL argument");
  CK(cudaSetDevice(ctx->device));
  NEED(ctx->params_set, DPMM_ESTATE, "set_params must precede debug_loglik");
  NEED(which == 0 || which == 1, DPMM_EINVAL, "which must be 0 or 1");
  const size_t cols = which == 0 ? (size_t)ctx->K : 2;
  float* dump = nullptr;
  CK(cudaMalloc((void**)&dump, cols * ctx->n * 4));
  int rc = 0;
  if (which == 0) {
    int32_t* keep = ctx->labels;
    int32_t* scratch = nullptr;
    const uint32_t call0 = ctx->call;
    const int lb0 = ctx->label_bound;
    if (cudaMalloc((void**)&scratch, (size_t)ctx->n * 4) != cudaSuccess) {
      cudaFree(dump);
      return fail(ctx, DPMM_ECUDA, "cudaMalloc(scratch labels) failed");
    }
    ctx->labels = scratch;
    rc = run_sample_labels(ctx, 1, dump);
    cudaStreamSynchronize(ctx->stream);
    ctx->labels = keep;
    ctx->call = call0;
    ctx->label_bound = lb0;
    ctx->hist_valid = ctx->scan_valid = ctx->sorted = ctx->partitioned = ctx->stats_cached = false;
    cudaFree(scratch);
  } else {
    uint8_t* keep = nullptr;
    const uint32_t call0 = ctx->call;
    if (ctx->label_bound > ctx->K) {
      cudaFree(dump);
      return fail(ctx, DPMM_ESTATE, "labels refer to clusters beyond the K of set_params");
    }
    if (cudaMalloc((void**)&keep, (size_t)ctx->n) != cudaSuccess) {
      cudaFree(dump);
      return fail(ctx, DPMM_ECUDA, "cudaMalloc(scratch sub-labels) failed");
    }
    cudaMemcpyAsync(keep, ctx->sub, (size_t)ctx->n, cudaMemcpyDeviceToDevice, ctx->stream);
    rc = run_sublabels(ctx, true, dump);
    cudaMemcpyAsync(ctx->sub, keep, (size_t)ctx->n, cudaMemcpyDeviceToDevice, ctx->stream);
    cudaStreamSynchronize(ctx->stream);
    ctx->call = call0;
    ctx->partitioned = ctx->stats_cached = false;
    cudaFree(keep);
  }
  if (rc == 0) {
    cudaError_t e = cudaMemcpy(out, dump, cols * ctx->n * 4, cudaMemcpyDeviceToHost);
    if (e != cudaSuccess) rc = fail(ctx, DPMM_ECUDA, std::string("cudaMemcpy(dump): ") + cudaGetErrorString(e));
  }
  cudaFree(dump);
  return rc;
}

extern "C" int dpmm_debug_tc_stats(dpmm_ctx* ctx, int64_t* out3) {
  NEED(ctx && out3, DPMM_EINVAL, "NULL argument");
  CK(cudaSetDevice(ctx->device));
  out3[0] = out3[1] = out3[2] = 0;
  if (ctx->tc_stats == nullptr) return 0;
  int32_t h[2] = {0, 0};
  CK(cudaStreamSynchronize(ctx->stream));
  CK(cudaMemcpy(h, ctx->tc_stats, 8, cudaMemcpyDeviceToHost));
  out3[0] = h[0];
  out3[1] = h[1];
  if (ctx->t2_ctr != nullptr) {
    CK(cudaMemcpy(h, ctx->t2_ctr, 4, cudaMemcpyDeviceToHost));
    out3[2] = h[0];
  }
  return 0;
}

extern "C" int dpmm_debug_fused_stats(dpmm_ctx* ctx, int64_t* out3) {
  NEED(ctx && out3, DPMM_EINVAL, "NULL argument");
  out3[0] = ctx->n_fused;
  out3[1] = ctx->n_cached;
  out3[2] = ctx->n_recompute;
  return 0;
}

extern "C" int dpmm_timing_kinds(void) { return TK_COUNT; }
extern "C" const char* dpmm_timing_name(int32_t kind) { return (kind >= 0 && kind < TK_COUNT) ? kTimingNames[kind] : ""; }
extern "C" int64_t dpmm_launch_count(const dpmm_ctx* ctx) { return ctx ? ctx->launches : 0; }

static void drain_timers(dpmm_ctx* ctx) {
  for (auto& t : ctx->tev) {
    float ms = 0.f;
    if (cudaEventElapsedTime(&ms, t.a, t.b) == cudaSuccess) ctx->t_ms[t.kind] += ms;
    ctx->ev_pool.push_back(t.a);
    ctx->ev_pool.push_back(t.b);
  }
  ctx->tev.clear();
}

extern "C" int dpmm_timing_enable(dpmm_ctx* ctx, int32_t on) {
  NEED(ctx, DPMM_EINVAL, "ctx is NULL");
  CK(cudaSetDevice(ctx->device));
  CK(cudaStreamSynchronize(ctx->stream));
  drain_timers(ctx);
  ctx->timing = on != 0;
  return 0;
}

extern "C" int dpmm_timing_read(dpmm_ctx* ctx, double* ms, int64_t* launches, int32_t reset) {
  NEED(ctx, DPMM_EINVAL, "ctx is NULL");
  CK(cudaSetDevice(ctx->device));
  CK(cudaStreamSynchronize(ctx->stream));
  drain_timers(ctx);
  for (int k = 0; k < TK_COUNT; ++k) {
    if (ms) ms[k] = ctx->t_ms[k];
    if (launches) launches[k] = ctx->t_n[k];
    if (reset) {
      ctx->t_ms[k] = 0;
      ctx->t_n[k] = 0;
    }
  }
  return 0;
}

static int load_nccl(dpmm_ctx* ctx, NcclApi& api) {
  if (api.handle) return 0;
  const char* names[] = {"libnccl.so.2", "libnccl.so"};
  for (const char* nm : names) {
    api.handle = dlopen(nm, RTLD_NOW | RTLD_GLOBAL);
    if (api.handle) break;
  }
  if (!api.handle) return fail(ctx, DPMM_ENCCL, std::string("dlopen(libnccl.so.2) failed: ") + dlerror());
  api.GetUniqueId = (decltype(api.GetUniqueId))dlsym(api.handle, "ncclGetUniqueId");
  api.CommInitRank = (decltype(api.CommInitRank))dlsym(api.handle, "ncclCommInitRank");
  api.AllReduce = (decltype(api.AllReduce))dlsym(api.handle, "ncclAllReduce");
  api.AllGather = (decltype(api.AllGather))dlsym(api.handle, "ncclAllGather");
  api.CommDestroy = (decltype(api.CommDestroy))dlsym(api.handle, "ncclCommDestroy");
  api.GetErrorString = (decltype(api.GetErrorString))dlsym(api.handle, "ncclGetErrorString");
  if (!api.GetUniqueId || !api.CommInitRank || !api.AllReduce || !api.CommDestroy || !api.GetErrorString)
    return fail(ctx, DPMM_ENCCL, "libnccl is missing a required symbol");
  return 0;
}

extern "C" int dpmm_nccl_unique_id(void* out128) {
  dpmm_ctx* ctx = nullptr;
  NEED(out128, DPMM_EINVAL, "out128 is NULL");
  static NcclApi api;
  int rc = load_nccl(nullptr, api);
  if (rc) return rc;
  const int r = api.GetUniqueId(out128);
  if (r != 0) return fail(nullptr, DPMM_ENCCL, std::string("ncclGetUniqueId: ") + api.GetErrorString(r));
  return 0;
}

extern "C" int dpmm_comm_init(dpmm_ctx* ctx, const void* unique_id128, int32_t rank, int32_t world_size) {
  NEED(ctx && unique_id128, DPMM_EINVAL, "NULL argument");
  NEED(world_size >= 1 && rank >= 0 && rank < world_size, DPMM_EINVAL, "bad rank / world size");
  CK(cudaSetDevice(ctx->device));
  int rc = load_nccl(ctx, ctx->nccl);
  if (rc) return rc;
// ... 48 lines not shown
```

dpmmsubclusters.jl_b200/csrc/kernels_gauss_tc2.cuh:

```cuda
#pragma once
#include "tcgen05.cuh"
#include "kernels_gauss.cuh"
#include "kernels_stats.cuh"

#define T2_TILE 128
#define T2_PRODUCERS(D) ((D) == 32 ? 128 : 64)
#define T2_THREADS(D) (320 + T2_PRODUCERS(D))
#define T2_CMAX 8
#define T2_R 8
#define T2_DELTA 30.0f
#define T2_MAX_K 256
#define T2_COOP_MAX 12
#define T2_NS32 4

struct GaussTc2Args {
  const float* x;
  int64_t n;
  int K, KS, nch, n0;
  const int32_t* perm;
  const int32_t* seg_off;
  int nkeys;
  const float* wpiv;
  const float* wscr;
  const float* wbias;
  const float* urows;
  const float* mu;
  const float* cst;
  const float* logw;
  const float* fro;
  const float* fro8;
  int32_t* labels;
  int32_t* hist;
  int32_t* ovf_list;
  int32_t* ovf_count;
  const double* u_inj;
  uint64_t seed;
  uint32_t call;
  int64_t goff;
  int final_iter;
  int32_t* stats;
};

struct GaussTc2Smem {
  int ns, pf;
  size_t stage_bytes, piv_bytes, scr_bytes, bias_bytes;
  size_t stages, piv, scr, bias, aaug, ccfro, scrc, cfin, lists, rlists, pairs, misc, bnd, pre, hist, bars, total;
  __host__ __device__ GaussTc2Smem(int D, int K, int KS, int nch, int nkeys) {
    ns = D == 32 ? T2_NS32 : 3;
    pf = ns - 2;
    stage_bytes = (size_t)T2_TILE * D * 4;
    piv_bytes = (size_t)(D * D) * 4;
    scr_bytes = (size_t)(KS / 8) * 4096;
    bias_bytes = (size_t)nch * 2048 + 128;
    size_t o = 0;
    stages = o;  o += ns * stage_bytes;
    piv = o;     o += 2 * piv_bytes;
    scr = o;     o += (size_t)nch * scr_bytes;
    bias = o;    o += 2 * bias_bytes;
    aaug = o;    o += 4096;
    ccfro = o;   o += (size_t)K * 8;
    o = (o + 15) & ~(size_t)15;
    scrc = o;    o += (size_t)(nch * 8 + 8) * 16;
    cfin = o;    o += (size_t)K * 8;
    o = (o + 15) & ~(size_t)15;
    lists = o;   o += 2 * T2_TILE * T2_CMAX * 2;
    rlists = o;  o += 2 * T2_TILE * T2_CMAX * 4;
    pairs = o;   o += 2 * T2_TILE * T2_CMAX * 2;
    misc = o;    o += 2 * 16 * 4;
    bnd = o;     o += (size_t)(nkeys + 1) * 4;
    pre = o;     o += (size_t)(nkeys + 1) * 4;
    hist = o;    o += (size_t)((K + 3) & ~3) * 4;
    o = (o + 15) & ~(size_t)15;
    bars = o;    o += 32 * 8 + 16;
    total = o;
  }
};
__host__ __device__ inline int gauss_tc2_n0(int D) { return (128 - D) / T2_R; }
__host__ __device__ inline int gauss_tc2_nch(int D, int K) {
  const int n0 = gauss_tc2_n0(D);
  return K <= n0 ? 1 : 1 + (K - n0 + 15) / 16;
}

#define T2_ROUNDS 8
#define T2_SEG_MIN 32
struct T2Seq {
  const int32_t* B;
  const int32_t* P;
  int nkeys, ntot, G, cta, R;
};
struct T2Walk {
  int key, pos, end, tleft;
  int t, send, seg;
};
__device__ __forceinline__ int t2_seg_begin(const T2Seq& q, int seg) {
  return (int)(((int64_t)q.ntot * seg) / ((int64_t)q.G * q.R));
}
__device__ __forceinline__ int t2_cta_tiles(const T2Seq& q) {
  int n = 0;
  for (int r = 0; r < q.R; ++r) n += t2_seg_begin(q, q.cta + r * q.G + 1) - t2_seg_begin(q, q.cta + r * q.G);
  return n;
}
__device__ __forceinline__ void t2_seek(T2Walk& w, const T2Seq& q, int t) {
  int lo = 0, hi = q.nkeys - 1;
  while (lo < hi) {
    const int mid = (lo + hi) >> 1;
    if (q.P[mid + 1] > t) hi = mid;
    else lo = mid + 1;
  }
  w.key = lo;
  w.pos = q.B[lo] + (t - q.P[lo]) * T2_TILE;
  w.end = q.B[lo + 1];
  w.t = t;
}
__device__ __forceinline__ void t2_enter(T2Walk& w, const T2Seq& q, int seg) {
  int b = t2_seg_begin(q, seg), e = t2_seg_begin(q, seg + 1);
  while (e <= b) {
    seg += q.G;
    b = t2_seg_begin(q, seg);
    e = t2_seg_begin(q, seg + 1);
  }
  w.seg = seg;
  w.send = e;
  t2_seek(w, q, b);
// ... 98 lines not shown
    rs[j] = e;
    s = __fadd_rn(s, e);
  }
  const bool s_regular = (s > 0.f) && (s < CUDART_INF_F);
  float cw = 0.f;
  for (int j = 0; j < m; ++j) {
    const float e = rs[j];
    const bool zero = (e < 1.17549435e-38f) && s_regular;
    const float quo = __fdiv_rn(zero ? 1.f : e, s);
    cw = __fadd_rn(cw, zero ? 0.f : quo);
    rs[j] = cw;
  }
  const double t = u * (double)cw;
  if (!(0.0 < t) && ks[0] != 0) return 0;
  for (int j = 0; j < m; ++j) {
    const int k = ks[j];
    if (k >= K - 1) break;
    if (!((double)rs[j] < t)) return k;
  }
  return K - 1;
}

__device__ __forceinline__ float t2_sum8(const uint32_t* v) {
  const f32x2_t p0 = f2_pack(__uint_as_float(v[0]), __uint_as_float(v[1]));
  const f32x2_t p1 = f2_pack(__uint_as_float(v[2]), __uint_as_float(v[3]));
  const f32x2_t p2 = f2_pack(__uint_as_float(v[4]), __uint_as_float(v[5]));
  const f32x2_t p3 = f2_pack(__uint_as_float(v[6]), __uint_as_float(v[7]));
  f32x2_t a0 = f2_fma(p0, p0, 0ull), a1 = f2_fma(p1, p1, 0ull);
  a0 = f2_fma(p2, p2, a0);
  a1 = f2_fma(p3, p3, a1);
  float x0, x1, y0, y1;
  f2_unpack(a0, x0, x1);
  f2_unpack(a1, y0, y1);
  return (x0 + x1) + (y0 + y1);
}

template <int D>
__global__ void __launch_bounds__(T2_THREADS(D), 1) gauss_label_tc2_kernel(const GaussTc2Args a) {
  extern __shared__ __align__(1024) uint8_t t2_smem[];
  uint8_t* const smem = t2_smem;
  const int K = a.K, KS = a.KS, nch = a.nch, n0 = a.n0, nkeys = a.nkeys;
  const GaussTc2Smem L(D, K, KS, nch, nkeys);
  constexpr int NS = D == 32 ? T2_NS32 : 3;
  constexpr int PF = NS - 2;
  constexpr int PIVF = D * D;
  uint8_t* stage0 = smem + L.stages;
  float* pivsm = reinterpret_cast<float*>(smem + L.piv);
  float* scrsm = reinterpret_cast<float*>(smem + L.scr);
  float* aaug = reinterpret_cast<float*>(smem + L.aaug);
  float2* ccfro = reinterpret_cast<float2*>(smem + L.ccfro);
  float4* scrc = reinterpret_cast<float4*>(smem + L.scrc);
  uint8_t* biassm = smem + L.bias;
  float2* cfin = reinterpret_cast<float2*>(smem + L.cfin);
  uint16_t* lists_all = reinterpret_cast<uint16_t*>(smem + L.lists);
  float* rl_all = reinterpret_cast<float*>(smem + L.rlists);
  uint16_t* pairs_all = reinterpret_cast<uint16_t*>(smem + L.pairs);
  int32_t* B = reinterpret_cast<int32_t*>(smem + L.bnd);
  int32_t* P = reinterpret_cast<int32_t*>(smem + L.pre);
  int* hs = reinterpret_cast<int*>(smem + L.hist);
  uint64_t* bars = reinterpret_cast<uint64_t*>(smem + L.bars);
  uint64_t* full = bars;
  uint64_t* empty = bars + 8;
  uint64_t* tfull = bars + 16;
  uint64_t* tempty = bars + 20;
  uint64_t* wdone = bars + 24;
  uint32_t* tmem_ptr = reinterpret_cast<uint32_t*>(bars + 32);

  const int tid = threadIdx.x, lane = tid & 31, warp = tid >> 5;

  if (tid == 0) {
    for (int i = 0; i < NS; ++i) {
      tc::mbar_init(&full[i], T2_PRODUCERS(D));
      tc::mbar_init(&empty[i], 128);
    }
    for (int i = 0; i < 4; ++i) {
      tc::mbar_init(&tfull[i], 1);
      tc::mbar_init(&tempty[i], 128);
    }
    tc::mbar_init(&wdone[0], 1);
    tc::mbar_init(&wdone[1], 1);
    tc::fence_barrier_init();
  }
  if (warp == 1) tc::tmem_alloc(tmem_ptr, 512);
  for (int j = tid; j <= nkeys; j += T2_THREADS(D)) B[j] = __ldg(a.seg_off + j);
  {
    const int nf4 = nch * (KS / 8) * 256;
    const float4* src = reinterpret_cast<const float4*>(a.wscr);
    float4* dst = reinterpret_cast<float4*>(scrsm);
    for (int e = tid; e < nf4; e += T2_THREADS(D)) dst[e] = __ldg(src + e);
  }
  for (int e = tid; e < 1024; e += T2_THREADS(D)) aaug[e] = 0.f;
  for (int k = tid; k < K; k += T2_THREADS(D)) {
    const float c = __ldg(a.cst + 3 * k), lw = __ldg(a.logw + k);
    ccfro[k] = make_float2(lw - c, __ldg(a.fro + k));
    cfin[k] = make_float2(c, lw);
    hs[k] = 0;
  }
  for (int e = tid; e < nch * 16 + 16; e += T2_THREADS(D)) {
    const int ch = e >> 4, j = e & 15;
    const int k = ch == 0 ? (j < n0 ? j : K) : n0 + (ch - 1) * 16 + j;
    float* q = reinterpret_cast<float*>(scrc + (e >> 1)) + (e & 1);
    q[0] = k < K ? 4.0816f * (__ldg(a.logw + k) - __ldg(a.cst + 3 * k)) : -CUDART_INF_F;
    q[2] = k < K ? __ldg(a.fro8 + k) : 0.f;
  }
  __syncthreads();
  for (int r = tid; r < T2_TILE; r += T2_THREADS(D)) {
    float* p = aaug + (r >> 3) * 64 + (r & 7) * 4;
    p[0] = 1.f;
    p[1] = 1.f;
  }
  if (warp == 0) {
    int carry = 0;
    if (lane == 0) P[0] = 0;
    for (int base = 0; base < nkeys; base += 32) {
      const int j = base + lane;
      int v = j < nkeys ? (B[j + 1] - B[j] + T2_TILE - 1) / T2_TILE : 0;
#pragma unroll
      for (int o = 1; o < 32; o <<= 1) {
        const int u = __shfl_up_sync(0xffffffffu, v, o);
        if (lane >= o) v += u;
      }
      if (j < nkeys) P[j + 1] = carry + v;
      carry += __shfl_sync(0xffffffffu, v, 31);
    }
  }
  tc::fence_proxy_async();
  tc::tc_fence_before();
  __syncthreads();
  tc::tc_fence_after();
  const uint32_t tmem_base = *tmem_ptr;
  const int ntot = P[nkeys];
  const T2Seq seq{B, P, nkeys, ntot, (int)gridDim.x, (int)blockIdx.x,
                  min(T2_ROUNDS, max(1, ntot / ((int)gridDim.x * T2_SEG_MIN)))};
  const int nt = t2_cta_tiles(seq);

  if (nt > 0) {
    if (warp < 2) {
      const int g = warp;
      const uint32_t tmem_u = __shfl_sync(0xffffffffu, tmem_base, 0);
      float* pivs = pivsm + (size_t)g * PIVF;
      float* biasg = reinterpret_cast<float*>(biassm + (size_t)g * L.bias_bytes);
      const int bias_f4 = (int)(L.bias_bytes / 16);
      const uint32_t pivs_a = tc::smem_u32(pivs), scr_a = tc::smem_u32(scrsm), bias_a = tc::smem_u32(biasg);
      const uint64_t aaug_desc = tc::smem_desc_k_noswz(tc::smem_u32(aaug));
      const uint32_t scr_stride = (uint32_t)L.scr_bytes;
      T2Walk w;
      t2_walk_init(w, seq);
      uint32_t cc = 0;
      int prevkey = -1, ntile_g = 0;
      for (int li = 0; li < nt; ++li, t2_advance(w, seq)) {
        if ((li & 1) != g) continue;
        const int s = li % NS;
        const int key = min(w.key, K - 1);
        tc::mbar_wait(&full[s], (li / NS) & 1);
        tc::tc_fence_after();
        const uint32_t st_a = tc::smem_u32(stage0 + (size_t)s * L.stage_bytes);
        for (int c = 0; c < nch; ++c, ++cc) {
          const int b = cc & 1;
          tc::mbar_wait(&tempty[g * 2 + b], ((cc >> 1) & 1) ^ 1);
          tc::tc_fence_after();
          const uint32_t tmem_d = tmem_u + g * 256 + b * 128;
          int col = 0;
          if (c == 0) {
            if (key != prevkey) {
              if (ntile_g > 0) tc::mbar_wait(&wdone[g], (ntile_g - 1) & 1);
              const float4* src = reinterpret_cast<const float4*>(a.wpiv + (size_t)key * PIVF);
// ... 162 lines not shown
            const int k0 = kbase + b0 * 4;
            if ((unsigned)(key - k0) < 8u) h &= ~(1u << (key - k0));
            if (h) append(h, k0);
          }
          tc::tc_fence_before();
          tc::mbar_arrive(&tempty[g * 2 + b]);
        }
        bool multi = valid && !weird && cnt > 0 && cnt < T2_CMAX;
        bool ovf = valid && (weird || cnt >= T2_CMAX);
        if (multi) {
          int j = cnt;
          while (j > 0 && mylist[j - 1] > key) {
            mylist[j] = mylist[j - 1];
            --j;
          }
          mylist[j] = (uint16_t)key;
          ++cnt;
        }
        if (__any_sync(0xffffffffu, multi)) {
          const int mine = multi ? cnt : 0;
          int inc = mine;
#pragma unroll
          for (int o = 1; o < 32; o <<= 1) {
            const int t = __shfl_up_sync(0xffffffffu, inc, o);
            if (lane >= o) inc += t;
          }
          const int total = __shfl_sync(0xffffffffu, inc, 31), off = inc - mine;
          uint16_t* wpairs = pairs + wq * 32 * T2_CMAX;
          for (int j = 0; j < mine; ++j) wpairs[off + j] = (uint16_t)((row << 3) | j);
          __syncwarp();
          if (total <= T2_COOP_MAX) {
            for (int p = 0; p < total; ++p) {
              const int pr = wpairs[p], prow = pr >> 3, slot = pr & 7;
              const int k = lists[prow * T2_CMAX + slot];
              const int32_t pidx = __ldg(a.perm + w.pos + prow);
              const float q = gauss_tc2_exact_q_coop<D>(a.urows + (size_t)k * D * D, a.mu + (size_t)k * D, a.x + (size_t)pidx * D, lane);
              if (lane == 0) {
                const float2 cf = cfin[k];
                rl[prow * T2_CMAX + slot] = gauss_finish(cf.x, q, cf.y);
                ++ncand_total;
              }
            }
          } else {
            for (int p = lane; p < total; p += 32) {
              const int pr = wpairs[p], prow = pr >> 3, slot = pr & 7;
              const int k = lists[prow * T2_CMAX + slot];
              const int32_t pidx = __ldg(a.perm + w.pos + prow);
              const float q = gauss_tc2_exact_q_row<D>(a.urows + (size_t)k * D * D, a.mu + (size_t)k * D, a.x + (size_t)pidx * D);
              const float2 cf = cfin[k];
              rl[prow * T2_CMAX + slot] = gauss_finish(cf.x, q, cf.y);
              ++ncand_total;
            }
          }
          __syncwarp();
        }
        tc::mbar_arrive(&empty[s]);
        if (valid) {
          int lab = key;
          if (multi) {
            bool bad = false;
            for (int j = 0; j < cnt; ++j) bad |= (myrl[j] != myrl[j]);
            if (bad) {
              ovf = true;
            } else if (a.final_iter) {
              float bv = -CUDART_INF_F;
              lab = mylist[0];
              for (int j = 0; j < cnt; ++j)
                if (myrl[j] > bv) {
                  bv = myrl[j];
                  lab = mylist[j];
                }
            } else {
              const double u = dpmm_uniform(a.u_inj, idx, a.seed, DPMM_STREAM_LABEL, a.call, (uint64_t)(a.goff + idx));
              lab = gauss_tc2_draw_list(mylist, myrl, cnt, K, u);
            }
          } else if (!ovf) {
            if (a.u_inj != nullptr && lab > 0 && !a.final_iter && a.u_inj[idx] == 0.0) lab = 0;
          }
          if (ovf) {
            a.ovf_list[atomicAdd(a.ovf_count, 1)] = idx;
          } else {
            a.labels[idx] = lab;
            atomicAdd(&hs[lab], 1);
          }
          ++npts_total;
        }
      }
      {
#pragma unroll
        for (int o = 16; o > 0; o >>= 1) {
          npts_total += __shfl_xor_sync(0xffffffffu, npts_total, o);
          ncand_total += __shfl_xor_sync(0xffffffffu, ncand_total, o);
        }
        if (lane == 0 && a.stats != nullptr) {
          atomicAdd(&a.stats[0], npts_total);
          atomicAdd(&a.stats[1], ncand_total);
        }
      }
    } else {
      const int t64 = tid - 320;
      constexpr int CPR = D / 4;
      constexpr int RS = T2_PRODUCERS(D) / CPR;
      constexpr int NJ = T2_TILE / RS;
      const int c = t64 % CPR, r0 = t64 / CPR;
      T2Walk wl, wc;
      t2_walk_init(wl, seq);
      wc = wl;
      int ckey = -1;
      float4 cen = make_float4(0.f, 0.f, 0.f, 0.f);
      int32_t idx[NJ];
      auto load_idx = [&]() {
#pragma unroll
        for (int j = 0; j < NJ; ++j) {
          const int p = wl.pos + r0 + RS * j;
          idx[j] = p < wl.end ? __ldg(a.perm + p) : -1;
        }
      };
      if constexpr (D == 32) {
        static_assert(PF == 2, "one register set per tile in flight: va, vb");
        auto load_rows = [&](float4 (&v)[NJ]) {
#pragma unroll
          for (int j = 0; j < NJ; ++j) {
            const bool ok = idx[j] >= 0;
            v[j] = ldg_nc16(a.x + (size_t)(ok ? idx[j] : 0) * D + 4 * c, ok);
          }
        };
        float4 va[NJ], vb[NJ];
        load_idx();
        load_rows(va);
        t2_advance(wl, seq);
        if (1 < nt) {
          load_idx();
          load_rows(vb);
          t2_advance(wl, seq);
        }
        if (2 < nt) load_idx();
        auto tile = [&](int li, float4 (&v)[NJ]) {
          const int key = min(wc.key, K - 1);
          if (key != ckey) {
            ckey = key;
            cen = __ldg(reinterpret_cast<const float4*>(a.mu + (size_t)key * D) + c);
          }
          const int nrow = wc.end - wc.pos;
          t2_advance(wc, seq);
#pragma unroll
          for (int j = 0; j < NJ; ++j) {
            if (r0 + RS * j < nrow) {
              v[j].x -= cen.x; v[j].y -= cen.y; v[j].z -= cen.z; v[j].w -= cen.w;
            }
          }
          tc::mbar_wait(&empty[li % NS], ((li / NS) & 1) ^ 1);
          uint8_t* base = stage0 + (size_t)(li % NS) * L.stage_bytes;
#pragma unroll
          for (int j = 0; j < NJ; ++j) {
            const int r = r0 + RS * j;
            *reinterpret_cast<float4*>(base + r * 128 + ((c ^ (r & 7)) << 4)) = v[j];
          }
          tc::fence_proxy_async();
          tc::mbar_arrive(&full[li % NS]);
          const int nx = li + PF;
          if (nx < nt) {
            load_rows(v);
            t2_advance(wl, seq);
            if (nx + 1 < nt) load_idx();
          }
        };
// ... 1 lines not shown
          tile(li, va);
          if (li + 1 < nt) tile(li + 1, vb);
        }
      } else {
        auto issue = [&](int s) {
          uint8_t* dst0 = stage0 + (size_t)s * L.stage_bytes + (c >> 3) * 16384;
#pragma unroll
          for (int j = 0; j < NJ; ++j) {
            const int r = r0 + RS * j;
            const bool ok = idx[j] >= 0;
            cp_async16(dst0 + r * 128 + (((c & 7) ^ (r & 7)) << 4), a.x + (size_t)(ok ? idx[j] : 0) * D + 4 * c, ok ? 16 : 0);
          }
        };
        load_idx();
#pragma unroll
        for (int q = 0; q < PF; ++q) {
          if (q < nt) {
            issue(q % NS);
            t2_advance(wl, seq);
            if (q + 1 < nt) load_idx();
          }
          cp_async_commit();
        }
        for (int li = 0; li < nt; ++li) {
          cp_async_wait_group<PF - 1>();
          {
            const int key = min(wc.key, K - 1);
            if (key != ckey) {
              ckey = key;
              cen = __ldg(reinterpret_cast<const float4*>(a.mu + (size_t)key * D) + c);
            }
            uint8_t* base = stage0 + (size_t)(li % NS) * L.stage_bytes + (c >> 3) * 16384;
            const int nrow = wc.end - wc.pos;
#pragma unroll
            for (int j = 0; j < NJ; ++j) {
              const int r = r0 + RS * j;
              float4* q = reinterpret_cast<float4*>(base + r * 128 + (((c & 7) ^ (r & 7)) << 4));
              float4 v = *q;
              if (r < nrow) {
                v.x -= cen.x; v.y -= cen.y; v.z -= cen.z; v.w -= cen.w;
                *q = v;
              }
            }
            t2_advance(wc, seq);
          }
          tc::fence_proxy_async();
          tc::mbar_arrive(&full[li % NS]);
          const int nx = li + PF;
          if (nx < nt) {
            tc::mbar_wait(&empty[nx % NS], ((nx / NS) & 1) ^ 1);
            issue(nx % NS);
            t2_advance(wl, seq);
            if (nx + 1 < nt) load_idx();
          }
          cp_async_commit();
        }
      }
    }
  }
  tc::tc_fence_before();
  __syncthreads();
  if (warp == 1) tc::tmem_dealloc(tmem_base, 512);
  for (int k = tid; k < K; k += T2_THREADS(D))
    if (hs[k] != 0) atomicAdd(&a.hist[k], hs[k]);
}

struct GaussListArgs {
  const float* x;
  int K;
  const int32_t* list;
  const int32_t* count;
  const float* urows;
  const float* mu;
  const float* cst;
  const float* logw;
  int32_t* labels;
  int32_t* hist;
  const double* u_inj;
  uint64_t seed;
  uint32_t call;
  int64_t goff;
  int final_iter;
  int32_t* stats;
  int32_t* zero_next;
  int32_t* ticket;
  int scan_k;
  int32_t* seg_off;
  int32_t* scat_cursor;
  int32_t* lr_cursor;
};

template <int D>
__global__ void __launch_bounds__(256) gauss_label_list_kernel(const GaussListArgs a) {
  extern __shared__ float gl_rs[];
  const int lane = threadIdx.x & 31, wl = threadIdx.x >> 5;
  const int nlist = *a.count;
  if (a.zero_next != nullptr && blockIdx.x == 0 && threadIdx.x < 4) a.zero_next[threadIdx.x] = 0;
  float* rs = gl_rs + (size_t)wl * a.K;
  for (int e = blockIdx.x * 8 + wl; e < nlist; e += gridDim.x * 8) {
    const int32_t idx = a.list[e];
    const float* xr = a.x + (size_t)idx * D;
    for (int k = lane; k < a.K; k += 32) {
      const float q = gauss_tc2_exact_q_impl<D>(a.urows + (size_t)k * D * D, a.mu + (size_t)k * D,
                                                [&](int c) { return __ldg(reinterpret_cast<const float4*>(xr) + c); });
      rs[k] = gauss_finish(__ldg(a.cst + 3 * k), q, __ldg(a.logw + k));
    }
    __syncwarp();
    if (lane == 0) {
      int lab;
      if (a.final_iter) {
        lab = dpmm_draw_argmax(rs, 1, a.K);
      } else {
        const double u = dpmm_uniform(a.u_inj, idx, a.seed, DPMM_STREAM_LABEL, a.call, (uint64_t)(a.goff + idx));
        lab = dpmm_draw_inverse_cdf(rs, 1, a.K, u);
      }
      a.labels[idx] = lab;
      atomicAdd(a.hist + lab, 1);
      if (a.stats != nullptr) atomicAdd(&a.stats[1], a.K);
    }
    __syncwarp();
  }
  if (a.ticket != nullptr) {
    __shared__ int last_block;
    __shared__ int wtot[8];
    __threadfence();
    __syncthreads();
    if (threadIdx.x == 0) last_block = atomicAdd(a.ticket, 1) == (int)gridDim.x - 1;
    __syncthreads();
    if (last_block) {
      __threadfence();
      int carry = 0;
      for (int k0 = 0; k0 < a.scan_k; k0 += 256) {
        const int k = k0 + (int)threadIdx.x;
        const int v = k < a.scan_k ? __ldcg(a.hist + k) : 0;
        int inc = v;
#pragma unroll
        for (int o = 1; o < 32; o <<= 1) {
          const int t = __shfl_up_sync(0xffffffffu, inc, o);
          if (lane >= o) inc += t;
        }
        if (lane == 31) wtot[wl] = inc;
        __syncthreads();
        int before = 0, total = 0;
#pragma unroll
        for (int w = 0; w < 8; ++w) {
          before += w < wl ? wtot[w] : 0;
          total += wtot[w];
        }
        const int excl = carry + before + inc - v;
        if (k < a.scan_k) {
          a.seg_off[k] = excl;
          a.scat_cursor[k] = excl;
          a.lr_cursor[2 * k] = excl;
          a.lr_cursor[2 * k + 1] = excl + v;
        }
        carry += total;
        __syncthreads();
      }
      if (threadIdx.x == 0) {
        a.seg_off[a.scan_k] = carry;
        *a.ticket = 0;
      }
    }
  }
}
```

dpmmsubclusters.jl_b200/csrc/kernels_sort.cuh:

```cuda
#pragma once
#include "common.cuh"

__global__ void label_hist_kernel(const int32_t* __restrict__ labels, int64_t n, int K, int32_t* hist) {
  extern __shared__ int hs[];
  for (int k = threadIdx.x; k < K; k += blockDim.x) hs[k] = 0;
  __syncthreads();
  for (int64_t i = (int64_t)blockIdx.x * blockDim.x + threadIdx.x; i < n; i += (int64_t)gridDim.x * blockDim.x) {
    const int l = labels[i];
    if (l >= 0 && l < K) atomicAdd(&hs[l], 1);
  }
  __syncthreads();
  for (int k = threadIdx.x; k < K; k += blockDim.x)
    if (hs[k] != 0) atomicAdd(&hist[k], hs[k]);
}

__global__ void label_scan_kernel(const int32_t* __restrict__ hist, int K, int32_t* seg_off,
                                  int32_t* scat_cursor, int32_t* lr_cursor) {
  __shared__ int warp_tot[32];
  __shared__ int carry;
  const int tid = threadIdx.x, lane = tid & 31, wid = tid >> 5;
  if (tid == 0) carry = 0;
  __syncthreads();
  for (int k0 = 0; k0 < K; k0 += blockDim.x) {
    const int k = k0 + tid;
    const int v = (k < K) ? hist[k] : 0;
    int inc = v;
#pragma unroll
    for (int o = 1; o < 32; o <<= 1) {
      const int t = __shfl_up_sync(0xffffffffu, inc, o);
      if (lane >= o) inc += t;
    }
    if (lane == 31) warp_tot[wid] = inc;
    __syncthreads();
    if (wid == 0) {
      int w = (lane < (blockDim.x >> 5)) ? warp_tot[lane] : 0;
#pragma unroll
      for (int o = 1; o < 32; o <<= 1) {
        const int t = __shfl_up_sync(0xffffffffu, w, o);
        if (lane >= o) w += t;
      }
      warp_tot[lane] = w;
    }
    __syncthreads();
    const int excl = carry + (wid ? warp_tot[wid - 1] : 0) + inc - v;
    if (k < K) {
      seg_off[k] = excl;
      scat_cursor[k] = excl;
      lr_cursor[2 * k] = excl;
      lr_cursor[2 * k + 1] = excl + v;
    }
    __syncthreads();
    if (tid == 0) carry += warp_tot[(blockDim.x >> 5) - 1];
    __syncthreads();
  }
  if (tid == 0) seg_off[K] = carry;
}

#define SCATTER_PPT 8
__global__ void label_scatter_kernel(const int32_t* __restrict__ labels, int64_t n, int K,
                                     int32_t* cursor, int32_t* perm, double* zero, int64_t nzero,
                                     int32_t* zero2, int nzero2) {
  extern __shared__ int sm[];
  for (int64_t e = (int64_t)blockIdx.x * blockDim.x + threadIdx.x; e < nzero; e += (int64_t)gridDim.x * blockDim.x) zero[e] = 0.0;
  for (int e = blockIdx.x * blockDim.x + threadIdx.x; e < nzero2; e += gridDim.x * blockDim.x) zero2[e] = 0;
  int* cnt = sm;
  int* basev = sm + K;
  const int T = blockDim.x, tid = threadIdx.x;
  for (int k = tid; k < K; k += T) cnt[k] = 0;
  __syncthreads();
  const int64_t base = (int64_t)blockIdx.x * T * SCATTER_PPT;
  int lab[SCATTER_PPT], rank[SCATTER_PPT];
#pragma unroll
  for (int j = 0; j < SCATTER_PPT; ++j) {
    const int64_t i = base + (int64_t)j * T + tid;
    lab[j] = (i < n) ? labels[i] : -1;
  }
#pragma unroll
  for (int j = 0; j < SCATTER_PPT; ++j) {
    const int lane = tid & 31;
    const int lab0 = __shfl_sync(0xffffffffu, lab[j], 0);
    if (__all_sync(0xffffffffu, lab[j] == lab0)) {
      int b0 = 0;
      if (lane == 0 && lab0 >= 0) b0 = atomicAdd(&cnt[lab0], 32);
      rank[j] = __shfl_sync(0xffffffffu, b0, 0) + lane;
    } else if (lab[j] >= 0) {
      rank[j] = atomicAdd(&cnt[lab[j]], 1);
    }
  }
  __syncthreads();
  for (int k = tid; k < K; k += T) {
    const int c = cnt[k];
    basev[k] = c ? atomicAdd(&cursor[k], c) : 0;
  }
  __syncthreads();
#pragma unroll
  for (int j = 0; j < SCATTER_PPT; ++j) {
    const int64_t i = base + (int64_t)j * T + tid;
    if (lab[j] >= 0) perm[basev[lab[j]] + rank[j]] = (int32_t)i;
  }
}

__global__ void relabel_kernel(int32_t* labels, uint8_t* sub, int64_t n, int K,
                               const int32_t* __restrict__ lut_l, const int32_t* __restrict__ lut_r,
                               const uint8_t* __restrict__ rule, const uint8_t* r_inj, uint64_t seed,
                               uint32_t call, int64_t goff) {
  for (int64_t i = (int64_t)blockIdx.x * blockDim.x + threadIdx.x; i < n; i += (int64_t)gridDim.x * blockDim.x) {
    const int k = labels[i];
    if (k < 0 || k >= K) continue;
    const int s = sub[i];
    const int nk = s ? lut_r[k] : lut_l[k];
    if (nk != k) labels[i] = nk;
    const int r = rule[k];
    if (r == 1) sub[i] = 0;
    else if (r == 2) sub[i] = 1;
    else if (r == 3) sub[i] = (uint8_t)dpmm_randbit(r_inj, i, seed, call, (uint64_t)(goff + i));
  }
}

__global__ void init_labels_kernel(int32_t* labels, int64_t n, int init_clusters, int shift,
                                   uint64_t seed, uint32_t call, int64_t goff) {
  for (int64_t i = (int64_t)blockIdx.x * blockDim.x + threadIdx.x; i < n; i += (int64_t)gridDim.x * blockDim.x) {
    const double u = philox_to_uniform(philox_draw(seed, DPMM_STREAM_INIT, call, (uint64_t)(goff + i)));
    int l = (int)(u * (double)init_clusters);
    if (l > init_clusters - 1) l = init_clusters - 1;
    labels[i] = l + shift;
  }
}

template <typename T>
__global__ void widen_labels_kernel(const T* __restrict__ in, int64_t n, int64_t* __restrict__ out) {
  for (int64_t i = (int64_t)blockIdx.x * blockDim.x + threadIdx.x; i < n; i += (int64_t)gridDim.x * blockDim.x)
    out[i] = (int64_t)in[i] + 1;
}
template <typename T>
__global__ void narrow_labels_kernel(const int64_t* __restrict__ in, int64_t n, int64_t hi, T* __restrict__ out,
                                     int32_t* __restrict__ status) {
  int mx = 0, bad = 0;
  for (int64_t i = (int64_t)blockIdx.x * blockDim.x + threadIdx.x; i < n; i += (int64_t)gridDim.x * blockDim.x) {
    const int64_t v = in[i];
    if (v < 1 || v > hi) bad = 1;
    else {
      out[i] = (T)(v - 1);
      mx = max(mx, (int)v);
    }
  }
#pragma unroll
  for (int o = 16; o > 0; o >>= 1) {
// ... 26 lines not shown
```

dpmmsubclusters.jl_b200/csrc/kernels_stats.cuh:

```cuda
#pragma once
#include "common.cuh"

struct StatsItem {
  int32_t key;
  int32_t begin;
  int32_t end;
};

#ifndef DPMM_TEMPLATES_ONLY
__global__ void stats_worklist_kernel(const int32_t* __restrict__ seg_off, const int32_t* __restrict__ lr_cursor,
                                      const uint8_t* __restrict__ wanted, int K, int chunk, StatsItem* items,
                                      int32_t* n_items, int32_t* next_item) {
  extern __shared__ int sc[];
  const int tid = threadIdx.x;
  for (int key = tid; key < 2 * K; key += blockDim.x) {
    const int k = key >> 1;
    int len = 0;
    if (wanted == nullptr || wanted[k]) {
      const int mid = lr_cursor[2 * k];
      len = (key & 1) ? seg_off[k + 1] - mid : mid - seg_off[k];
    }
    sc[key] = (len + chunk - 1) / chunk;
  }
  __syncthreads();
// ... 289 lines not shown
        int t = e - D, i = 0;
        while (t >= D - i) {
          t -= D - i;
          ++i;
        }
        if (v[s] != 0.f) atomicAdd(dst + D + (size_t)i * D + (i + t), (double)v[s]);
      }
    }
  }
}

#ifndef DPMM_TEMPLATES_ONLY
#define MNM_STATS_NREG 32
#define MNM_STATS_UNROLL 8
template <bool SLICED>
__global__ void __launch_bounds__(256) mnm_stats_kernel(const StatsArgs a) {
  const int lane = threadIdx.x & 31;
  const int nslices = SLICED ? (a.D + 32 * MNM_STATS_NREG - 1) / (32 * MNM_STATS_NREG) : 1;
  const int n_units = *a.n_items * nslices;
  for (;;) {
    int u = 0;
    if (lane == 0) u = atomicAdd(a.next_item, 1);
    u = __shfl_sync(0xffffffffu, u, 0);
    if (u >= n_units) break;
    const StatsItem item = a.items[u / nslices];
    {
      const int d0 = (u % nslices) * 32 * MNM_STATS_NREG;
      const int D = SLICED ? min(a.D - d0, 32 * MNM_STATS_NREG) : a.D;
      const float* x = a.x + d0;
      const int nreg = (D + 31) >> 5;
      float acc[MNM_STATS_NREG];
#pragma unroll
      for (int r = 0; r < MNM_STATS_NREG; ++r) acc[r] = 0.f;
      int idx_n[MNM_STATS_UNROLL];
#pragma unroll
      for (int j = 0; j < MNM_STATS_UNROLL; ++j) idx_n[j] = (item.begin + j < item.end) ? __ldg(a.perm2 + item.begin + j) : -1;
      for (int p0 = item.begin; p0 < item.end; p0 += MNM_STATS_UNROLL) {
        int idx[MNM_STATS_UNROLL];
#pragma unroll
        for (int j = 0; j < MNM_STATS_UNROLL; ++j) {
          idx[j] = idx_n[j];
          const int pn = p0 + MNM_STATS_UNROLL + j;
          idx_n[j] = (pn < item.end) ? __ldg(a.perm2 + pn) : -1;
        }
        if (nreg <= 4) {
          float v[MNM_STATS_UNROLL][4];
#pragma unroll
          for (int j = 0; j < MNM_STATS_UNROLL; ++j)
#pragma unroll
            for (int r = 0; r < 4; ++r) {
              const int d = lane + 32 * r;
              v[j][r] = (idx[j] >= 0 && d < D) ? __ldg(x + (size_t)idx[j] * a.D + d) : 0.f;
            }
#pragma unroll
          for (int j = 0; j < MNM_STATS_UNROLL; ++j)
#pragma unroll
            for (int r = 0; r < 4; ++r) acc[r] += v[j][r];
        } else {
#pragma unroll
          for (int j = 0; j < MNM_STATS_UNROLL; ++j)
            if (idx[j] >= 0) {
#pragma unroll
              for (int r = 0; r < MNM_STATS_NREG; ++r) {
                const int d = lane + 32 * r;
                if (r < nreg && d < D) acc[r] += __ldg(x + (size_t)idx[j] * a.D + d);
              }
            }
        }
      }
      double* dst = a.acc + (size_t)item.key * a.rec + 1 + d0;
#pragma unroll
      for (int r = 0; r < MNM_STATS_NREG; ++r) {
        const int d = lane + 32 * r;
        if (r < nreg && d < D && acc[r] != 0.f) atomicAdd(dst + d, (double)acc[r]);
      }
    }
  }
}

__global__ void stats_finalize_kernel(const double* __restrict__ acc, const int32_t* __restrict__ seg_off,
                                      const int32_t* __restrict__ lr_cursor, const int32_t* __restrict__ idx_list,
                                      int m, int D, int rec, int niw, double* out, const float* __restrict__ centers,
                                      const int32_t* __restrict__ lcount, double* risk) {
  const int a = blockIdx.y;
  if (a >= m) return;
  const int k = idx_list != nullptr ? idx_list[a] : a;
  const double* L = acc + (size_t)(2 * k) * rec;
  const double* R = acc + (size_t)(2 * k + 1) * rec;
  const int beg = seg_off[k], end = seg_off[k + 1];
  const int mid = lcount != nullptr ? beg + lcount[k] : lr_cursor[2 * k];
  const double nl = (double)(mid - beg), nr = (double)(end - mid);
  const float* cl = centers != nullptr ? centers + (size_t)(2 * k) * D : nullptr;
  const float* cr = centers != nullptr ? centers + (size_t)(2 * k + 1) * D : nullptr;
  for (int e = blockIdx.x * blockDim.x + threadIdx.x; e < rec; e += gridDim.x * blockDim.x) {
    double l, r;
    if (e == 0) {
      l = nl;
      r = nr;
    } else if (e <= D || !niw) {
      l = L[e];
      r = R[e];
      if (cl != nullptr) l += nl * (double)cl[e - 1];
      if (cr != nullptr) r += nr * (double)cr[e - 1];
    } else {
      const int q = e - 1 - D;
      int i = q / D, j = q - i * D;
      if (i > j) {
        const int t = i;
        i = j;
        j = t;
      }
      l = L[1 + D + (size_t)i * D + j];
      r = R[1 + D + (size_t)i * D + j];
      if (cl != nullptr) {
        const double ci = cl[i], cj = cl[j], l0 = l;
        l += ci * L[1 + j] + L[1 + i] * cj + nl * ci * cj;
        if (risk != nullptr && i == j && nl > 0 && l0 > 32.0 * l) atomicAdd(risk, 1.0);
      }
      if (cr != nullptr) {
        const double ci = cr[i], cj = cr[j], r0 = r;
        r += ci * R[1 + j] + R[1 + i] * cj + nr * ci * cj;
        if (risk != nullptr && i == j && nr > 0 && r0 > 32.0 * r) atomicAdd(risk, 1.0);
      }
    }
    double* o = out + (size_t)a * 3 * rec;
    o[e] = l + r;
    o[rec + e] = l;
    o[2 * rec + e] = r;
  }
}

#endif
```

dpmmsubclusters.jl_b200/csrc/kernels_substats_tc.cuh:

```cuda
#pragma once
#include "kernels_gauss.cuh"
#include "kernels_stats_tc.cuh"

#define SS_D 32
#define SS_TILE 128
#define SS_RAW 5
#define SS_PF 2
#define SS_NG 3
#define SS_FLUSH 8
#define SS_NTB 6
#define SS_THREADS 896
#define SS_GATHER 256
#define SS_PANEL 16384
#define SS_PROWS 136
#define SS_PPANEL (SS_PROWS * 128)
#define SS_WSLOT (8192 + 8192 + 2048)
#define SS_TMEM_COLS 512
#define SS_TMEM_G2 (SS_NTB * 64)
#define SS_TLD 65

struct SubStatsArgs {
  const float* x;
  int64_t n;
  int K;
  const int32_t* perm;
  const int32_t* seg_off;
  const float* w;
  const float* bias;
  const float* cen;
  const float* cst;
  const float* loglr;
  uint8_t* sub;
  double* acc;
  int rec;
  int32_t* lcount;
  float* centers;
  const double* u_inj;
  uint64_t seed;
  uint32_t call;
  int64_t goff;
  float* dump;
};

struct SubStatsSmem {
  size_t raw, split, perm, wslot, aaug, tbuf, tri, dest, cnt, kcnt, bnd, pre, bars, slot, total;
  __host__ __device__ explicit SubStatsSmem(int K) {
    size_t o = 0;
    raw = o;    o += (size_t)SS_RAW * SS_PANEL;
    split = o;  o += (size_t)2 * SS_PANEL;
    perm = o;   o += (size_t)2 * 2 * SS_PPANEL;
    wslot = o;  o += (size_t)SS_WSLOT;
    aaug = o;   o += 4096;
    tbuf = o;   o += 64 * SS_TLD * 4;
    tri = o;    o += 528 * 2;
    o = (o + 15) & ~(size_t)15;
    dest = o;   o += SS_NG * SS_TILE;
    cnt = o;    o += SS_NG * 4 * 4;
    kcnt = o;   o += 4 * 4;
    bnd = o;    o += (size_t)(K + 1) * 4;
    pre = o;    o += (size_t)(K + 1) * 4;
    o = (o + 15) & ~(size_t)15;
    bars = o;   o += 40 * 8;
    slot = o;   o += 16;
    total = o;
  }
};

__global__ void __launch_bounds__(SS_THREADS, 1) niw_substats_tc_kernel(const SubStatsArgs a) {
  extern __shared__ __align__(1024) uint8_t ss_smem[];
  const SubStatsSmem L(a.K);
  uint8_t* raw0 = ss_smem + L.raw;
  uint8_t* split0 = ss_smem + L.split;
  uint8_t* perm0 = ss_smem + L.perm;
  uint8_t* wslot = ss_smem + L.wslot;
  float* aaug = reinterpret_cast<float*>(ss_smem + L.aaug);
  float* T = reinterpret_cast<float*>(ss_smem + L.tbuf);
  uint16_t* tri = reinterpret_cast<uint16_t*>(ss_smem + L.tri);
  uint8_t* dest_s = ss_smem + L.dest;
  volatile int32_t* cnt_s = reinterpret_cast<int32_t*>(ss_smem + L.cnt);
  volatile int32_t* kcnt = reinterpret_cast<int32_t*>(ss_smem + L.kcnt);
  int32_t* B = reinterpret_cast<int32_t*>(ss_smem + L.bnd);
  int32_t* P = reinterpret_cast<int32_t*>(ss_smem + L.pre);
  uint64_t* bars = reinterpret_cast<uint64_t*>(ss_smem + L.bars);
  uint64_t* ready = bars;
  uint64_t* sfree = bars + 2;
  uint64_t* landed = bars + 18;
  uint64_t* rfree = bars + 23;
  uint64_t* d1full = bars + 28;
  uint64_t* d1empty = bars + 34;
  uint64_t* permd = bars + 8;
  uint64_t* pfree = bars + 4;
  uint64_t* d2full = bars + 12;
  uint64_t* d2empty = bars + 14;
  uint64_t* wfull = bars + 16;
  uint64_t* wempty = bars + 17;
  uint32_t* tmem_slot = reinterpret_cast<uint32_t*>(ss_smem + L.slot);
  const int tid = threadIdx.x, lane = tid & 31, warp = tid >> 5;
  const int nkeys = a.K;

  for (int j = tid; j <= nkeys; j += SS_THREADS) B[j] = __ldg(a.seg_off + j);
  for (int e = tid; e < 1024; e += SS_THREADS) {
    const int i = e >> 5, j = e & 31;
    if (j >= i) tri[i * 32 - (i * (i - 1)) / 2 + (j - i)] = (uint16_t)((i << 8) | j);
  }
  for (int e = tid; e < 1024; e += SS_THREADS) aaug[e] = 0.f;
  {
    float* baug = reinterpret_cast<float*>(wslot + 16384);
    for (int e = tid; e < 512; e += SS_THREADS) baug[e] = 0.f;
  }
  if (blockIdx.x == 0)
    for (int e = tid; e < 2 * nkeys * SS_D; e += SS_THREADS)
      a.centers[e] = __ldg(a.cen + (size_t)(e >> 6) * SS_D + (e & 31));
  if (tid == 0) {
    for (int b = 0; b < SS_NTB; ++b) {
      tc::mbar_init(&d1full[b], 1);
      tc::mbar_init(&d1empty[b], 128);
    }
    for (int b = 0; b < 2; ++b) {
      tc::mbar_init(&permd[b], 128);
      tc::mbar_init(&d2full[b], 2);
      tc::mbar_init(&d2empty[b], 128);
    }
    for (int b = 0; b < 4; ++b) tc::mbar_init(&pfree[b], 2);
    for (int r = 0; r < SS_RAW; ++r) {
      tc::mbar_init(&landed[r], SS_GATHER);
      tc::mbar_init(&rfree[r], 128);
    }
    for (int b = 0; b < 2; ++b) {
      tc::mbar_init(&ready[b], SS_GATHER);
      tc::mbar_init(&sfree[b], 1);
    }
    tc::mbar_init(wfull, 32);
    tc::mbar_init(wempty, 1);
    tc::fence_barrier_init();
  }
  __syncthreads();
  for (int r = tid; r < SS_TILE; r += SS_THREADS) {
    float* p = aaug + (r >> 3) * 64 + (r & 7) * 4;
    p[0] = 1.f;
    p[1] = 1.f;
  }
  if (warp == 0) {
    int carry = 0;
    if (lane == 0) P[0] = 0;
    for (int base = 0; base < nkeys; base += 32) {
      const int j = base + lane;
      int v = j < nkeys ? (B[j + 1] - B[j] + SS_TILE - 1) / SS_TILE : 0;
#pragma unroll
      for (int o = 1; o < 32; o <<= 1) {
        const int u = __shfl_up_sync(0xffffffffu, v, o);
        if (lane >= o) v += u;
      }
      if (j < nkeys) P[j + 1] = carry + v;
      carry += __shfl_sync(0xffffffffu, v, 31);
    }
  }
  if (warp == 4) tc::tmem_alloc(tmem_slot, SS_TMEM_COLS);
  tc::fence_proxy_async();
  tc::tc_fence_before();
  __syncthreads();
  tc::tc_fence_after();
  const uint32_t tmem_base = *tmem_slot;
  const int ntot = P[nkeys];
  const int t0 = (int)(((int64_t)ntot * blockIdx.x) / gridDim.x);
  const int t1 = (int)(((int64_t)ntot * (blockIdx.x + 1)) / gridDim.x);
  const int nt = t1 - t0;

  if (nt > 0) {
    if (warp < 4 || (warp >= 19 && warp < 23)) {
      const int gtid = warp < 4 ? tid : tid - 608 + 128;
      const int c = gtid & 7, r0 = gtid >> 3;
      const uint32_t offk = (uint32_t)(r0 * 128 + ((c ^ (r0 & 7)) << 4));
      const uint32_t offr = offk;
      StcWalk wl, wc;
      stc_walk_init(wl, B, P, nkeys, t0, t1);
      wc = wl;
      int idx[4];
      auto load_idx = [&]() {
#pragma unroll
        for (int j = 0; j < 4; ++j) {
          const int p = wl.pos + r0 + 32 * j;
          idx[j] = p < wl.end ? __ldg(a.perm + p) : -1;
        }
      };
      auto load_rows = [&](float4 (&v)[4]) {
#pragma unroll
        for (int j = 0; j < 4; ++j) {
          const bool ok = idx[j] >= 0;
          v[j] = ldg_nc16(a.x + (size_t)(ok ? idx[j] : 0) * SS_D + 4 * c, ok);
        }
      };
      float4 va[4], vb[4];
      load_idx();
      load_rows(va);
      stc_advance<SS_FLUSH>(wl, B);
      if (1 < nt) {
        load_idx();
        load_rows(vb);
        stc_advance<SS_FLUSH>(wl, B);
      }
      if (SS_PF < nt) load_idx();
      auto load_center = [&](int key) { return __ldg(reinterpret_cast<const float4*>(a.cen + (size_t)key * SS_D) + c); };
      int ckey = wc.key;
      float4 cen = load_center(ckey);
      auto tile = [&](int li, float4 (&v)[4]) {
        const int b = li & 1;
        if (wc.key != ckey) {
          ckey = wc.key;
          cen = load_center(ckey);
        }
        const int npts = wc.end - wc.pos;
#pragma unroll
        for (int j = 0; j < 4; ++j) {
          if (r0 + 32 * j < npts) {
            v[j].x -= cen.x; v[j].y -= cen.y; v[j].z -= cen.z; v[j].w -= cen.w;
          }
        }
        tc::mbar_wait(&rfree[li % SS_RAW], ((li / SS_RAW) & 1) ^ 1);
        uint8_t* zk = raw0 + (size_t)(li % SS_RAW) * SS_PANEL + offr;
#pragma unroll
        for (int j = 0; j < 4; ++j) *reinterpret_cast<float4*>(zk + j * 4096) = v[j];
        tc::mbar_arrive(&landed[li % SS_RAW]);
        tc::mbar_wait(&sfree[b], ((li >> 1) & 1) ^ 1);
        uint8_t* lk = split0 + (size_t)b * SS_PANEL + offk;
#pragma unroll
        for (int j = 0; j < 4; ++j) {
          float4 lo;
          lo.x = v[j].x - tc::trunc_tf32(v[j].x); lo.y = v[j].y - tc::trunc_tf32(v[j].y);
          lo.z = v[j].z - tc::trunc_tf32(v[j].z); lo.w = v[j].w - tc::trunc_tf32(v[j].w);
          *reinterpret_cast<float4*>(lk + j * 4096) = lo;
        }
        tc::fence_proxy_async();
        tc::mbar_arrive(&ready[b]);
        const int ln = li + SS_PF;
        if (ln < nt) {
          load_rows(v);
          stc_advance<SS_FLUSH>(wl, B);
          if (ln + 1 < nt) load_idx();
        }
        stc_advance<SS_FLUSH>(wc, B);
// ... 321 lines not shown
```

dpmmsubclusters.jl_b200/sweep.py:

```python
from __future__ import annotations

import ctypes as C

import numpy as np

from . import _lib as L

NIW = L.PRIOR_NIW
MULTINOMIAL = L.PRIOR_MULTINOMIAL


def _ptr(a, ctype):
    return None if a is None else a.ctypes.data_as(C.POINTER(ctype))


def _i64(a):
    return np.ascontiguousarray(np.asarray(a, dtype=np.int64))


class GpuSweep:

    def __init__(self, x, prior_kind, seed=0, global_offset=0, device=0):
        self.lib = L.load()
        x = np.asarray(x, dtype=np.float32)
# ... 175 lines not shown
                                                      _ptr(lr, C.c_float)))
        return lp, w, lr

    def predict_niw(self, u, mu, tconst, df, want_probs=True):
        u = np.ascontiguousarray(u, np.float32); mu = np.ascontiguousarray(mu, np.float32)
        tconst = np.ascontiguousarray(tconst, np.float32); df = np.ascontiguousarray(df, np.float32)
        K = u.shape[0]
        assert u.shape == (K, self.D, self.D) and mu.shape == (K, self.D) and tconst.shape == (K,) and df.shape == (K,)
        labels = np.empty(self.n, np.int64)
        probs = np.empty((self.n, K), np.float32) if want_probs else None
        self._ck(self.lib.dpmm_predict_niw(self.h, K, _ptr(u, C.c_float), _ptr(mu, C.c_float), _ptr(tconst, C.c_float),
                                           _ptr(df, C.c_float), _ptr(labels, C.c_int64), _ptr(probs, C.c_float)))
        return labels, probs

    def predict_multinomial(self, logp, logw, want_probs=True):
        logp = np.ascontiguousarray(logp, np.float64); logw = np.ascontiguousarray(logw, np.float32)
        K = logp.shape[0]
        assert logp.shape == (K, self.D) and logw.shape == (K,)
        labels = np.empty(self.n, np.int64)
        probs = np.empty((self.n, K), np.float32) if want_probs else None
        self._ck(self.lib.dpmm_predict_multinomial(self.h, K, _ptr(logp, C.c_double), _ptr(logw, C.c_float),
                                                   _ptr(labels, C.c_int64), _ptr(probs, C.c_float)))
        return labels, probs

    def smart_project(self, cluster, v, mu):
        v = np.ascontiguousarray(v, np.float64); mu = np.ascontiguousarray(mu, np.float64)
        assert v.shape == (self.D,) and mu.shape == (self.D,)
        lohi = np.empty(2, np.float64)
        cnt = np.zeros(1, np.int64)
        self._ck(self.lib.dpmm_smart_project(self.h, int(cluster), _ptr(v, C.c_double), _ptr(mu, C.c_double),
                                             _ptr(lohi, C.c_double), _ptr(cnt, C.c_int64)))
        return float(lohi[0]), float(lohi[1]), int(cnt[0])

    def smart_kmeans_iter(self, min_mean, max_mean):
        out = np.empty(4, np.float64)
        self._ck(self.lib.dpmm_smart_kmeans_iter(self.h, float(min_mean), float(max_mean), _ptr(out, C.c_double)))
        return tuple(float(o) for o in out)

    def smart_set_sublabels(self, cluster):
        self._ck(self.lib.dpmm_smart_set_sublabels(self.h, int(cluster)))

    def apply_split(self, indices, new_indices):
        a, b = _i64(indices), _i64(new_indices)
        assert len(a) == len(b)
        self._ck(self.lib.dpmm_apply_split(self.h, _ptr(a, C.c_int64), _ptr(b, C.c_int64), len(a)))

    def apply_merge(self, indices, new_indices):
        a, b = _i64(indices), _i64(new_indices)
        assert len(a) == len(b)
        self._ck(self.lib.dpmm_apply_merge(self.h, _ptr(a, C.c_int64), _ptr(b, C.c_int64), len(a)))

    def remove_empty(self, pts_count):
        a = _i64(pts_count)
        self._ck(self.lib.dpmm_remove_empty(self.h, _ptr(a, C.c_int64), len(a)))

    @staticmethod
    def nccl_unique_id():
        lib = L.load()
        buf = (C.c_char * 128)()
        L.check(lib.dpmm_nccl_unique_id(C.cast(buf, C.c_void_p)), None)
        return bytes(buf)

    def comm_init(self, unique_id: bytes, rank: int, world_size: int):
        buf = C.create_string_buffer(unique_id, 128)
        self._ck(self.lib.dpmm_comm_init(self.h, C.cast(buf, C.c_void_p), int(rank), int(world_size)))

    def set_uniforms(self, u_label=None, u_sub=None, r_bits=None):
        ul = None if u_label is None else np.ascontiguousarray(u_label, np.float64)
        us = None if u_sub is None else np.ascontiguousarray(u_sub, np.float64)
        rb = None if r_bits is None else np.ascontiguousarray(r_bits, np.uint8)
        self._ck(self.lib.dpmm_set_uniforms(self.h, _ptr(ul, C.c_double), _ptr(us, C.c_double), _ptr(rb, C.c_uint8)))

    def debug_loglik(self, which=0):
        cols = self.K if which == 0 else 2
        out = np.empty((cols, self.n), np.float32)
        self._ck(self.lib.dpmm_debug_loglik(self.h, int(which), _ptr(out, C.c_float)))
        return np.ascontiguousarray(out.T)

    def tc_stats(self, overflow=False):
        out = np.zeros(3, np.int64)
        self._ck(self.lib.dpmm_debug_tc_stats(self.h, _ptr(out, C.c_int64)))
        return (int(out[0]), int(out[1]), int(out[2])) if overflow else (int(out[0]), int(out[1]))

    def fused_stats(self):
        out = np.zeros(3, np.int64)
        self._ck(self.lib.dpmm_debug_fused_stats(self.h, _ptr(out, C.c_int64)))
        return int(out[0]), int(out[1]), int(out[2])

    def timing_enable(self, on=True):
        self._ck(self.lib.dpmm_timing_enable(self.h, 1 if on else 0))

    def timing_read(self, reset=True):
        nk = self.lib.dpmm_timing_kinds()
        ms = np.zeros(nk, np.float64)
        cnt = np.zeros(nk, np.int64)
        self._ck(self.lib.dpmm_timing_read(self.h, _ptr(ms, C.c_double), _ptr(cnt, C.c_int64), 1 if reset else 0))
        return {self.lib.dpmm_timing_name(i).decode(): (float(ms[i]), int(cnt[i])) for i in range(nk)}

    def launch_count(self):
        return int(self.lib.dpmm_launch_count(self.h))
```

include/dpmm_b200.h:

```cpp
#ifndef DPMM_B200_H
#define DPMM_B200_H

#include <stdint.h>

#ifdef __cplusplus
extern "C" {
#endif

#define DPMM_OK 0
#define DPMM_EINVAL (-1)
#define DPMM_ECUDA (-2)
#define DPMM_ESTATE (-3)
#define DPMM_ELIMIT (-4)
#define DPMM_ENCCL (-5)

#define DPMM_PRIOR_NIW 0
#define DPMM_PRIOR_MULTINOMIAL 1

#define DPMM_SAMPLER_INVERSE_CDF 0
#define DPMM_SAMPLER_GUMBEL 1

typedef struct dpmm_ctx dpmm_ctx;


int dpmm_create(dpmm_ctx** out, const float* x, int64_t n_local, int32_t d, int32_t prior_kind,
                int32_t device, uint64_t seed, int64_t global_offset);
int dpmm_destroy(dpmm_ctx* ctx);
const char* dpmm_last_error(const dpmm_ctx* ctx);
int dpmm_set_stream(dpmm_ctx* ctx, void* cuda_stream);
int dpmm_sync(dpmm_ctx* ctx);
int dpmm_limits(int32_t* out3);


int dpmm_init_labels(dpmm_ctx* ctx, int32_t init_clusters, int32_t outlier);
int dpmm_randomize_sublabels(dpmm_ctx* ctx, const int64_t* indices, int32_t n_indices);
int dpmm_get_labels(dpmm_ctx* ctx, int64_t* out);
int dpmm_get_sublabels(dpmm_ctx* ctx, int64_t* out);
int dpmm_set_labels(dpmm_ctx* ctx, const int64_t* labels);
int dpmm_set_sublabels(dpmm_ctx* ctx, const int64_t* sublabels);


int dpmm_set_params_niw(dpmm_ctx* ctx, int32_t k, const float* mu, const float* inv_sigma,
                        const float* logdet, const float* weights, const float* lr_weights);
int dpmm_set_params_multinomial(dpmm_ctx* ctx, int32_t k, const float* log_p, const float* weights,
                                const float* lr_weights);
int dpmm_set_sampler(dpmm_ctx* ctx, int32_t sampler);


int dpmm_sample_labels(dpmm_ctx* ctx, int32_t final_iter);
int dpmm_sample_sublabels(dpmm_ctx* ctx);
int dpmm_suff_stats(dpmm_ctx* ctx, const int64_t* indices, int32_t n_indices, int64_t* counts,
                    double* sum_x, double* sum_xx);

int dpmm_num_clusters(const dpmm_ctx* ctx);


int dpmm_set_hyper_niw(dpmm_ctx* ctx, double kappa, const double* m, double nu, const double* psi, double alpha);
int dpmm_set_hyper_multinomial(dpmm_ctx* ctx, const float* alpha_prior, double alpha);
int dpmm_posterior_step(dpmm_ctx* ctx, const int64_t* indices, int32_t n_indices, int32_t from_table,
                        const uint8_t* splittable, int32_t k_merge, int64_t* counts, double* logml,
                        double* merge_logml);
int dpmm_sample_params(dpmm_ctx* ctx, int32_t k, int32_t from_prior, int32_t unit_weights);
int dpmm_params_merge(dpmm_ctx* ctx, int64_t i, int64_t j);
int dpmm_get_params_niw(dpmm_ctx* ctx, int32_t k, float* mu, double* lfac, float* logdet, float* weights,
                        float* lr_weights);
int dpmm_get_params_multinomial(dpmm_ctx* ctx, int32_t k, float* log_p, float* weights, float* lr_weights);

int dpmm_predict_niw(dpmm_ctx* ctx, int32_t k, const float* u, const float* mu, const float* tconst,
                     const float* df, int64_t* labels, float* probs);
int dpmm_predict_multinomial(dpmm_ctx* ctx, int32_t k, const double* logp, const float* logw, int64_t* labels,
                             float* probs);


int dpmm_apply_split(dpmm_ctx* ctx, const int64_t* indices, const int64_t* new_indices, int32_t n);
int dpmm_apply_merge(dpmm_ctx* ctx, const int64_t* indices, const int64_t* new_indices, int32_t n);
int dpmm_remove_empty(dpmm_ctx* ctx, const int64_t* pts_count, int32_t k);


int dpmm_smart_project(dpmm_ctx* ctx, int64_t cluster, const double* v, const double* mu, double* lo_hi,
                       int64_t* count);
int dpmm_smart_kmeans_iter(dpmm_ctx* ctx, double min_mean, double max_mean, double* out4);
int dpmm_smart_set_sublabels(dpmm_ctx* ctx, int64_t cluster);


int dpmm_nccl_unique_id(void* out128);
int dpmm_comm_init(dpmm_ctx* ctx, const void* unique_id128, int32_t rank, int32_t world_size);


int dpmm_set_uniforms(dpmm_ctx* ctx, const double* u_label, const double* u_sub, const uint8_t* r_bits);
int dpmm_debug_loglik(dpmm_ctx* ctx, int32_t which, float* out);
int dpmm_debug_tc_stats(dpmm_ctx* ctx, int64_t* out3);
int dpmm_debug_fused_stats(dpmm_ctx* ctx, int64_t* out3);
int dpmm_timing_enable(dpmm_ctx* ctx, int32_t on);
int dpmm_timing_kinds(void);
const char* dpmm_timing_name(int32_t kind);
int dpmm_timing_read(dpmm_ctx* ctx, double* ms, int64_t* launches, int32_t reset);
int64_t dpmm_launch_count(const dpmm_ctx* ctx);

#ifdef __cplusplus
}
#endif
#endif
```

Baseline: 5359.

## Chain sweep kernels with PDL, fold memsets into kernels, skip unchanged scatter

Kernels in the label/scatter/substats/finalize chain now launch with programmatic dependent launch, and setup work (barrier init, TMEM alloc) is moved ahead of griddepcontrol.wait so it overlaps the previous kernel's tail. Several standalone memsets and the D2H stats copy are removed. The histogram is double-buffered and the spare copy is zeroed by the list kernel, and the host stats are written through mapped pinned memory. A device-side moved-label counter lets the scatter kernel exit early when no label changed. PDL for the TMEM-using kernels is enabled only when register footprints stop two of them sharing an SM, which adds bookkeeping and atomic traffic and risks subtle ordering bugs.

```diff
diff --git a/dpmmsubclusters.jl_b200/_lib.py b/dpmmsubclusters.jl_b200/_lib.py
--- a/dpmmsubclusters.jl_b200/_lib.py
+++ b/dpmmsubclusters.jl_b200/_lib.py
@@ -55,6 +55,7 @@
     "dpmm_set_uniforms": (C.c_int, [_p, _f64p, _f64p, _u8p]),
     "dpmm_debug_loglik": (C.c_int, [_p, _i32, _f32p]),
     "dpmm_debug_tc_stats": (C.c_int, [_p, _i64p]),
+    "dpmm_debug_sort": (C.c_int, [_p, C.POINTER(C.c_int32), _i64p]),
     "dpmm_debug_fused_stats": (C.c_int, [_p, _i64p]),
     "dpmm_timing_enable": (C.c_int, [_p, _i32]),
     "dpmm_timing_kinds": (C.c_int, []),
diff --git a/dpmmsubclusters.jl_b200/csrc/common.cuh b/dpmmsubclusters.jl_b200/csrc/common.cuh
--- a/dpmmsubclusters.jl_b200/csrc/common.cuh
+++ b/dpmmsubclusters.jl_b200/csrc/common.cuh
@@ -212,6 +212,25 @@
   return dpmm_draw_inverse_cdf(m, 1, 2, u);
 }
 
+__device__ __forceinline__ void pdl_wait() { asm volatile("griddepcontrol.wait;" ::: "memory"); }
+__device__ __forceinline__ void pdl_launch_dependents() { asm volatile("griddepcontrol.launch_dependents;" ::: "memory"); }
+
+template <typename... KArgs, typename... Args>
+inline cudaError_t launch_pdl(bool pdl, void (*kern)(KArgs...), dim3 grid, unsigned block, size_t smem,
+                              cudaStream_t stream, Args... args) {
+  cudaLaunchConfig_t cfg{};
+  cfg.gridDim = grid;
+  cfg.blockDim = dim3(block);
+  cfg.dynamicSmemBytes = smem;
+  cfg.stream = stream;
+  cudaLaunchAttribute attr[1];
+  attr[0].id = cudaLaunchAttributeProgrammaticStreamSerialization;
+  attr[0].val.programmaticStreamSerializationAllowed = 1;
+  cfg.attrs = attr;
+  cfg.numAttrs = pdl ? 1 : 0;
+  return cudaLaunchKernelEx(&cfg, kern, args...);
+}
+
 __device__ __forceinline__ double dpmm_uniform(const double* inj, int64_t local_i, uint64_t seed,
                                                uint32_t stream, uint32_t call, uint64_t gidx) {
   if (inj != nullptr) return inj[local_i];
diff --git a/dpmmsubclusters.jl_b200/csrc/ctx.cuh b/dpmmsubclusters.jl_b200/csrc/ctx.cuh
--- a/dpmmsubclusters.jl_b200/csrc/ctx.cuh
+++ b/dpmmsubclusters.jl_b200/csrc/ctx.cuh
@@ -103,6 +103,7 @@
   bool t2_params = false;
   int t2_KS = 0, t2_nch = 0;
   int32_t* t2_hstat = nullptr;
+  int32_t* t2_hstat_dev = nullptr;
   cudaEvent_t t2_hstat_ev = nullptr;
   bool t2_hstat_pending = false;
   int t2_cooldown = 0;
@@ -118,7 +119,13 @@
   bool tc_params = false;
   float* logp_t = nullptr;
   int KP = 0;
+  int32_t* hist_mem = nullptr;
   int32_t* hist = nullptr;
+  int hist_cur = 0;
+  int hist_spare_clean = 0;
+  const int32_t* t2_moved = nullptr;
+  int risk_zeroed_k = 0;
+  int pdl_tmem = -1;
   int32_t* seg_off = nullptr;
   int32_t* scat_cursor = nullptr;
   int32_t* lr_cursor = nullptr;
diff --git a/dpmmsubclusters.jl_b200/csrc/dpmm_b200.cu b/dpmmsubclusters.jl_b200/csrc/dpmm_b200.cu
--- a/dpmmsubclusters.jl_b200/csrc/dpmm_b200.cu
+++ b/dpmmsubclusters.jl_b200/csrc/dpmm_b200.cu
@@ -114,7 +114,11 @@
     CK(dev_realloc(&ctx->ss_b, (size_t)cap * 2 * D));
     CK(dev_realloc(&ctx->ss_c, (size_t)cap * D));
   }
-  CK(dev_realloc(&ctx->hist, (size_t)cap));
+  CK(dev_realloc(&ctx->hist_mem, (size_t)2 * cap));
+  ctx->hist = ctx->hist_mem;
+  ctx->hist_cur = ctx->hist_spare_clean = 0;
+  ctx->t2_moved = nullptr;
+  ctx->risk_zeroed_k = 0;
   CK(dev_realloc(&ctx->seg_off, (size_t)cap + 1));
   CK(dev_realloc(&ctx->scat_cursor, (size_t)cap));
   CK(dev_realloc(&ctx->lr_cursor, (size_t)2 * cap));
@@ -287,8 +291,8 @@
     }
   }
   if (ctx->tc_ok || (prior_kind == DPMM_PRIOR_NIW && (dpad == 32 || dpad == 64) && n_local >= T2_TILE)) {
-    CKC(cudaMalloc((void**)&ctx->ctr_sets, 8 * sizeof(int32_t)));
-    CKC(cudaMemset(ctx->ctr_sets, 0, 8 * sizeof(int32_t)));
+    CKC(cudaMalloc((void**)&ctx->ctr_sets, 2 * T2_CTR_SET * sizeof(int32_t)));
+    CKC(cudaMemset(ctx->ctr_sets, 0, 2 * T2_CTR_SET * sizeof(int32_t)));
     ctx->tc_stats = ctx->ctr_sets;
     ctx->t2_ctr = ctx->ctr_sets + 2;
   }
@@ -354,7 +358,7 @@
   }
   for (auto e : ctx->ev_pool) cudaEventDestroy(e);
   void* ptrs[] = {ctx->x, ctx->labels, ctx->sub, ctx->perm, ctx->perm2, ctx->u_label, ctx->u_sub, ctx->r_bits,
-                  ctx->raw_params, ctx->recs, ctx->cst, ctx->logw, ctx->loglr, ctx->logp_t, ctx->t2_piv, ctx->t2_scr, ctx->t2_u, ctx->t2_bias, ctx->t2_fro8, ctx->ctr_sets, ctx->tc_w, ctx->tc_b, ctx->tc_mu, ctx->tc_fro, ctx->ss_w, ctx->ss_b, ctx->ss_c, ctx->lcount, ctx->mtc_w, ctx->hist, ctx->seg_off,
+                  ctx->raw_params, ctx->recs, ctx->cst, ctx->logw, ctx->loglr, ctx->logp_t, ctx->t2_piv, ctx->t2_scr, ctx->t2_u, ctx->t2_bias, ctx->t2_fro8, ctx->ctr_sets, ctx->tc_w, ctx->tc_b, ctx->tc_mu, ctx->tc_fro, ctx->ss_w, ctx->ss_b, ctx->ss_c, ctx->lcount, ctx->mtc_w, ctx->hist_mem, ctx->seg_off,
                   ctx->scat_cursor, ctx->lr_cursor, ctx->lut_l, ctx->lut_r, ctx->rule, ctx->wanted,
                   ctx->idx_list, ctx->acc, ctx->centers, ctx->outbuf, ctx->items, ctx->item_ctr, ctx->hyper_d, ctx->ptab,
                   ctx->ptab_alt, ctx->post, ctx->post_alt, ctx->lfac, ctx->pm_out, ctx->splittable_d, ctx->newof_d,
@@ -822,6 +826,27 @@
 
 static int ensure_sorted(dpmm_ctx* ctx);
 
+static bool sweep_pdl_ok(dpmm_ctx* ctx) {
+  if (ctx->pdl_tmem < 0) {
+    const struct { const void* f; int threads; } ks[] = {{(const void*)gauss_label_tc2_kernel<32>, T2_THREADS(32)},
+                                                        {(const void*)gauss_label_tc2_kernel<64>, T2_THREADS(64)},
+                                                        {(const void*)niw_substats_tc_kernel, SS_THREADS}};
+    int regs_sm = 0;
+    bool ok = cudaDeviceGetAttribute(&regs_sm, cudaDevAttrMaxRegistersPerMultiprocessor, ctx->device) == cudaSuccess;
+    int foot[3];
+    for (int i = 0; i < 3 && ok; ++i) {
+      cudaFuncAttributes fa;
+      ok = cudaFuncGetAttributes(&fa, ks[i].f) == cudaSuccess;
+      foot[i] = fa.numRegs * ks[i].threads;
+    }
+    for (int i = 0; i < 3 && ok; ++i)
+      for (int j = 0; j < 3; ++j) ok &= foot[i] + foot[j] > regs_sm;
+    cudaGetLastError();
+    ctx->pdl_tmem = ok ? 1 : 0;
+  }
+  return ctx->pdl_tmem == 1 && !ctx->timing;
+}
+
 template <int D>
 static int launch_label_tc2(dpmm_ctx* ctx, int final_iter, int nkeys) {
   const int K = ctx->K;
@@ -831,39 +856,43 @@
   a.wbias = ctx->t2_bias; a.fro8 = ctx->t2_fro8;
   a.urows = ctx->t2_u; a.mu = ctx->tc_mu; a.cst = ctx->cst; a.logw = ctx->logw; a.fro = ctx->tc_fro;
   ctx->ctr_cur ^= 1;
-  ctx->tc_stats = ctx->ctr_sets + 4 * ctx->ctr_cur;
+  ctx->tc_stats = ctx->ctr_sets + T2_CTR_SET * ctx->ctr_cur;
   ctx->t2_ctr = ctx->tc_stats + 2;
   a.labels = ctx->labels; a.hist = ctx->hist; a.ovf_list = ctx->perm2; a.ovf_count = ctx->t2_ctr;
   a.u_inj = ctx->u_label; a.seed = ctx->seed; a.call = ctx->call; a.goff = ctx->goff; a.final_iter = final_iter;
   a.stats = ctx->tc_stats;
+  a.moved = ctx->tc_stats + 4;
   const size_t sm = GaussTc2Smem(D, K, a.KS, a.nch, nkeys).total;
   CK(cudaFuncSetAttribute(gauss_label_tc2_kernel<D>, cudaFuncAttributeMaxDynamicSharedMemorySize, (int)sm));
-  if (!ctx->ctr_clean) CK(cudaMemsetAsync(ctx->ctr_sets, 0, 8 * sizeof(int32_t), ctx->stream));
+  if (!ctx->ctr_clean) CK(cudaMemsetAsync(ctx->ctr_sets, 0, 2 * T2_CTR_SET * sizeof(int32_t), ctx->stream));
+  if (ctx->t2_hstat == nullptr) {
+    CK(cudaHostAlloc((void**)&ctx->t2_hstat, 4 * sizeof(int32_t), cudaHostAllocMapped));
+    CK(cudaHostGetDevicePointer((void**)&ctx->t2_hstat_dev, ctx->t2_hstat, 0));
+    CK(cudaEventCreateWithFlags(&ctx->t2_hstat_ev, cudaEventDisableTiming));
+  }
   const int64_t grid = std::min<int64_t>((ctx->n + T2_TILE - 1) / T2_TILE, (int64_t)ctx->sm_count);
   {
     KernelTimer kt(ctx, TK_LABEL);
-    gauss_label_tc2_kernel<D><<<(unsigned)grid, T2_THREADS(D), sm, ctx->stream>>>(a);
-    CK(cudaGetLastError());
+    CK(launch_pdl(sweep_pdl_ok(ctx), gauss_label_tc2_kernel<D>, (unsigned)grid, T2_THREADS(D), sm, ctx->stream, a));
   }
   GaussListArgs l{};
   l.x = ctx->x; l.K = K; l.list = ctx->perm2; l.count = ctx->t2_ctr; l.urows = ctx->t2_u; l.mu = ctx->tc_mu;
   l.cst = ctx->cst; l.logw = ctx->logw; l.labels = ctx->labels; l.hist = ctx->hist; l.u_inj = ctx->u_label;
   l.seed = ctx->seed; l.call = ctx->call; l.goff = ctx->goff; l.final_iter = final_iter; l.stats = a.stats;
-  l.zero_next = ctx->ctr_sets + 4 * (ctx->ctr_cur ^ 1);
+  l.moved = a.moved;
+  l.zero_next = ctx->ctr_sets + T2_CTR_SET * (ctx->ctr_cur ^ 1);
   ctx->ctr_clean = true;
+  l.zero_hist = ctx->hist_mem + (size_t)(ctx->hist_cur ^ 1) * ctx->Kcap;
+  l.zero_hist_n = K;
+  ctx->hist_spare_clean = K;
+  l.hstat = ctx->t2_hstat_dev;
   l.ticket = ctx->tc_stats + 3; l.scan_k = K; l.seg_off = ctx->seg_off; l.scat_cursor = ctx->scat_cursor; l.lr_cursor = ctx->lr_cursor;
   const size_t lsm = (size_t)8 * K * 4;
   if (lsm > 48 * 1024) CK(cudaFuncSetAttribute(gauss_label_list_kernel<D>, cudaFuncAttributeMaxDynamicSharedMemorySize, (int)lsm));
   {
     KernelTimer kt(ctx, TK_LABEL_OVF);
-    gauss_label_list_kernel<D><<<(unsigned)ctx->sm_count * 2, 256, lsm, ctx->stream>>>(l);
-    CK(cudaGetLastError());
-  }
-  if (ctx->t2_hstat == nullptr) {
-    CK(cudaMallocHost((void**)&ctx->t2_hstat, 4 * sizeof(int32_t)));
-    CK(cudaEventCreateWithFlags(&ctx->t2_hstat_ev, cudaEventDisableTiming));
-  }
-  CK(cudaMemcpyAsync(ctx->t2_hstat, ctx->tc_stats, 12, cudaMemcpyDeviceToHost, ctx->stream));
+    CK(launch_pdl(!ctx->timing, gauss_label_list_kernel<D>, (unsigned)ctx->sm_count * 2, 256, lsm, ctx->stream, l));
+  }
   CK(cudaEventRecord(ctx->t2_hstat_ev, ctx->stream));
   ctx->t2_hstat_pending = true;
   return 0;
@@ -912,7 +941,13 @@
     int rc = ensure_sorted(ctx);
     if (rc) return rc;
   }
-  CK(cudaMemsetAsync(ctx->hist, 0, (size_t)K * 4, ctx->stream));
+  if (use_t2 && ctx->hist_spare_clean >= K) {
+    ctx->hist_cur ^= 1;
+    ctx->hist = ctx->hist_mem + (size_t)ctx->hist_cur * ctx->Kcap;
+    ctx->hist_spare_clean = 0;
+  } else {
+    CK(cudaMemsetAsync(ctx->hist, 0, (size_t)K * 4, ctx->stream));
+  }
   if (use_t2) {
     int rc = ctx->D == 32 ? launch_label_tc2<32>(ctx, final_iter, nkeys) : launch_label_tc2<64>(ctx, final_iter, nkeys);
     if (rc) return rc;
@@ -982,6 +1017,7 @@
   }
   ctx->hist_valid = true;
   ctx->scan_valid = use_t2;
+  ctx->t2_moved = use_t2 ? ctx->tc_stats + 4 : nullptr;
   ctx->sorted = false;
   ctx->partitioned = ctx->stats_cached = false;
   ctx->label_bound = K;
@@ -1008,16 +1044,18 @@
     label_scan_kernel<<<1, 1024, 0, ctx->stream>>>(ctx->hist, K, ctx->seg_off, ctx->scat_cursor, ctx->lr_cursor);
     CK(cudaGetLastError());
   }
+  const int32_t* moved = ctx->hist_valid && ctx->scan_valid ? ctx->t2_moved : nullptr;
+  ctx->t2_moved = nullptr;
   ctx->scan_valid = false;
   {
     const int T = 256;
     const unsigned grid = (unsigned)((ctx->n + (int64_t)T * SCATTER_PPT - 1) / ((int64_t)T * SCATTER_PPT));
     const bool pre = ctx->prior == DPMM_PRIOR_NIW && ctx->D == SS_D && ctx->tc_ok && ctx->lcount != nullptr;
-    label_scatter_kernel<<<grid, T, (size_t)K * 8, ctx->stream>>>(ctx->labels, ctx->n, K, ctx->scat_cursor, ctx->perm,
-                                                                  pre ? ctx->acc : nullptr, pre ? (int64_t)2 * K * ctx->stats_rec : 0,
-                                                                  pre ? ctx->lcount : nullptr, pre ? K : 0);
-    CK(cudaGetLastError());
+    CK(launch_pdl(!ctx->timing, label_scatter_kernel, grid, T, (size_t)K * 8, ctx->stream, (const int32_t*)ctx->labels,
+                  ctx->n, K, ctx->scat_cursor, ctx->perm, pre ? ctx->acc : nullptr, pre ? (int64_t)2 * K * ctx->stats_rec : (int64_t)0,
+                  pre ? ctx->lcount : nullptr, pre ? K : 0, pre ? ctx->outbuf + (size_t)K * 3 * ctx->stats_rec : nullptr, moved));
     ctx->acc_cleared = pre;
+    ctx->risk_zeroed_k = pre ? K : 0;
   }
   ctx->sorted = true;
   ctx->partitioned = ctx->stats_cached = false;
@@ -1058,8 +1096,7 @@
     CK(cudaFuncSetAttribute(niw_substats_tc_kernel, cudaFuncAttributeMaxDynamicSharedMemorySize, (int)smem));
     {
       KernelTimer kt(ctx, TK_SUBLABEL);
-      niw_substats_tc_kernel<<<ctx->sm_count, SS_THREADS, smem, ctx->stream>>>(f);
-      CK(cudaGetLastError());
+      CK(launch_pdl(sweep_pdl_ok(ctx), niw_substats_tc_kernel, (unsigned)ctx->sm_count, SS_THREADS, smem, ctx->stream, f));
     }
     ctx->partitioned = false;
     ctx->stats_cached = true;
@@ -1234,13 +1271,12 @@
     KernelTimer kt(ctx, TK_STATS_AUX);
     const int T = 256;
     dim3 grid((unsigned)std::min((rec + T - 1) / T, 64), (unsigned)m);
-    CK(cudaMemsetAsync(fin + (size_t)m * 3 * rec, 0, 8, ctx->stream));
-    stats_finalize_kernel<<<grid, T, 0, ctx->stream>>>(ctx->acc, ctx->seg_off, ctx->lr_cursor, all ? nullptr : ctx->idx_list, m, D, rec,
-                                                       ctx->prior == DPMM_PRIOR_NIW ? 1 : 0, fin,
-                                                       (stats_tc || stats_tc64 || cached) ? ctx->centers : nullptr,
-                                                       cached ? ctx->lcount : nullptr,
-                                                       cached ? fin + (size_t)m * 3 * rec : nullptr);
-    CK(cudaGetLastError());
+    if (!(fin == ctx->outbuf && m == ctx->risk_zeroed_k)) CK(cudaMemsetAsync(fin + (size_t)m * 3 * rec, 0, 8, ctx->stream));
+    ctx->risk_zeroed_k = 0;
+    CK(launch_pdl(!ctx->timing, stats_finalize_kernel, grid, T, 0, ctx->stream, (const double*)ctx->acc, (const int32_t*)ctx->seg_off,
+                  (const int32_t*)ctx->lr_cursor, (const int32_t*)(all ? nullptr : ctx->idx_list), m, D, rec,
+                  ctx->prior == DPMM_PRIOR_NIW ? 1 : 0, fin, (const float*)((stats_tc || stats_tc64 || cached) ? ctx->centers : nullptr),
+                  (const int32_t*)(cached ? ctx->lcount : nullptr), cached ? fin + (size_t)m * 3 * rec : nullptr));
   }
   if (use_ipc) {
     IpcReduceArgs ia{};
@@ -1779,6 +1815,24 @@
   return 0;
 }
 
+extern "C" int dpmm_debug_sort(dpmm_ctx* ctx, int32_t* perm, int64_t* moved) {
+  NEED(ctx && moved, DPMM_EINVAL, "NULL argument");
+  CK(cudaSetDevice(ctx->device));
+  moved[0] = 0;
+  if (perm != nullptr) {
+    int rc = ensure_sorted(ctx);
+    if (rc) return rc;
+  }
+  CK(cudaStreamSynchronize(ctx->stream));
+  if (perm != nullptr) CK(cudaMemcpy(perm, ctx->perm, (size_t)ctx->n * 4, cudaMemcpyDeviceToHost));
+  if (ctx->ctr_sets != nullptr) {
+    int32_t h = 0;
+    CK(cudaMemcpy(&h, ctx->tc_stats + 4, 4, cudaMemcpyDeviceToHost));
+    moved[0] = h;
+  }
+  return 0;
+}
+
 extern "C" int dpmm_debug_fused_stats(dpmm_ctx* ctx, int64_t* out3) {
   NEED(ctx && out3, DPMM_EINVAL, "NULL argument");
   out3[0] = ctx->n_fused;
diff --git a/dpmmsubclusters.jl_b200/csrc/kernels_gauss_tc2.cuh b/dpmmsubclusters.jl_b200/csrc/kernels_gauss_tc2.cuh
--- a/dpmmsubclusters.jl_b200/csrc/kernels_gauss_tc2.cuh
+++ b/dpmmsubclusters.jl_b200/csrc/kernels_gauss_tc2.cuh
@@ -4,6 +4,7 @@
 #include "kernels_stats.cuh"
 
 #define T2_TILE 128
+#define T2_CTR_SET 8
 #define T2_PRODUCERS(D) ((D) == 32 ? 128 : 64)
 #define T2_THREADS(D) (320 + T2_PRODUCERS(D))
 #define T2_CMAX 8
@@ -39,6 +40,7 @@
   int64_t goff;
   int final_iter;
   int32_t* stats;
+  int32_t* moved;
 };
 
 struct GaussTc2Smem {
@@ -303,6 +305,8 @@
     tc::fence_barrier_init();
   }
   if (warp == 1) tc::tmem_alloc(tmem_ptr, 512);
+  pdl_wait();
+  pdl_launch_dependents();
   for (int j = tid; j <= nkeys; j += T2_THREADS(D)) B[j] = __ldg(a.seg_off + j);
   {
     const int nf4 = nch * (KS / 8) * 256;
@@ -631,6 +635,7 @@
           } else {
             a.labels[idx] = lab;
             atomicAdd(&hs[lab], 1);
+            if (lab != w.key) atomicAdd(a.moved, 1);
           }
           ++npts_total;
         }
@@ -798,7 +803,11 @@
   int64_t goff;
   int final_iter;
   int32_t* stats;
+  int32_t* moved;
   int32_t* zero_next;
+  int32_t* zero_hist;
+  int zero_hist_n;
+  int32_t* hstat;
   int32_t* ticket;
   int scan_k;
   int32_t* seg_off;
@@ -810,8 +819,11 @@
 __global__ void __launch_bounds__(256) gauss_label_list_kernel(const GaussListArgs a) {
   extern __shared__ float gl_rs[];
   const int lane = threadIdx.x & 31, wl = threadIdx.x >> 5;
+  pdl_wait();
+  pdl_launch_dependents();
   const int nlist = *a.count;
-  if (a.zero_next != nullptr && blockIdx.x == 0 && threadIdx.x < 4) a.zero_next[threadIdx.x] = 0;
+  if (a.zero_next != nullptr && blockIdx.x == 0 && threadIdx.x < T2_CTR_SET) a.zero_next[threadIdx.x] = 0;
+  for (int k = blockIdx.x * blockDim.x + threadIdx.x; k < a.zero_hist_n; k += gridDim.x * blockDim.x) a.zero_hist[k] = 0;
   float* rs = gl_rs + (size_t)wl * a.K;
   for (int e = blockIdx.x * 8 + wl; e < nlist; e += gridDim.x * 8) {
     const int32_t idx = a.list[e];
@@ -830,6 +842,7 @@
         const double u = dpmm_uniform(a.u_inj, idx, a.seed, DPMM_STREAM_LABEL, a.call, (uint64_t)(a.goff + idx));
         lab = dpmm_draw_inverse_cdf(rs, 1, a.K, u);
       }
+      if (a.moved != nullptr && a.labels[idx] != lab) atomicAdd(a.moved, 1);
       a.labels[idx] = lab;
       atomicAdd(a.hist + lab, 1);
       if (a.stats != nullptr) atomicAdd(&a.stats[1], a.K);
@@ -876,6 +889,12 @@
       if (threadIdx.x == 0) {
         a.seg_off[a.scan_k] = carry;
         *a.ticket = 0;
+        if (a.hstat != nullptr) {
+          a.hstat[0] = __ldcg(a.stats + 0);
+          a.hstat[1] = __ldcg(a.stats + 1);
+          a.hstat[2] = __ldcg(a.count);
+          __threadfence_system();
+        }
       }
     }
   }
diff --git a/dpmmsubclusters.jl_b200/csrc/kernels_sort.cuh b/dpmmsubclusters.jl_b200/csrc/kernels_sort.cuh
--- a/dpmmsubclusters.jl_b200/csrc/kernels_sort.cuh
+++ b/dpmmsubclusters.jl_b200/csrc/kernels_sort.cuh
@@ -59,10 +59,14 @@
 #define SCATTER_PPT 8
 __global__ void label_scatter_kernel(const int32_t* __restrict__ labels, int64_t n, int K,
                                      int32_t* cursor, int32_t* perm, double* zero, int64_t nzero,
-                                     int32_t* zero2, int nzero2) {
+                                     int32_t* zero2, int nzero2, double* zero3, const int32_t* moved) {
   extern __shared__ int sm[];
+  pdl_wait();
+  pdl_launch_dependents();
   for (int64_t e = (int64_t)blockIdx.x * blockDim.x + threadIdx.x; e < nzero; e += (int64_t)gridDim.x * blockDim.x) zero[e] = 0.0;
   for (int e = blockIdx.x * blockDim.x + threadIdx.x; e < nzero2; e += gridDim.x * blockDim.x) zero2[e] = 0;
+  if (zero3 != nullptr && blockIdx.x == 0 && threadIdx.x == 0) *zero3 = 0.0;
+  if (moved != nullptr && *moved == 0) return;
   int* cnt = sm;
   int* basev = sm + K;
   const int T = blockDim.x, tid = threadIdx.x;
diff --git a/dpmmsubclusters.jl_b200/csrc/kernels_stats.cuh b/dpmmsubclusters.jl_b200/csrc/kernels_stats.cuh
--- a/dpmmsubclusters.jl_b200/csrc/kernels_stats.cuh
+++ b/dpmmsubclusters.jl_b200/csrc/kernels_stats.cuh
@@ -395,6 +395,8 @@
                                       const int32_t* __restrict__ lr_cursor, const int32_t* __restrict__ idx_list,
                                       int m, int D, int rec, int niw, double* out, const float* __restrict__ centers,
                                       const int32_t* __restrict__ lcount, double* risk) {
+  pdl_wait();
+  pdl_launch_dependents();
   const int a = blockIdx.y;
   if (a >= m) return;
   const int k = idx_list != nullptr ? idx_list[a] : a;
diff --git a/dpmmsubclusters.jl_b200/csrc/kernels_substats_tc.cuh b/dpmmsubclusters.jl_b200/csrc/kernels_substats_tc.cuh
--- a/dpmmsubclusters.jl_b200/csrc/kernels_substats_tc.cuh
+++ b/dpmmsubclusters.jl_b200/csrc/kernels_substats_tc.cuh
@@ -98,7 +98,6 @@
   const int tid = threadIdx.x, lane = tid & 31, warp = tid >> 5;
   const int nkeys = a.K;
 
-  for (int j = tid; j <= nkeys; j += SS_THREADS) B[j] = __ldg(a.seg_off + j);
   for (int e = tid; e < 1024; e += SS_THREADS) {
     const int i = e >> 5, j = e & 31;
     if (j >= i) tri[i * 32 - (i * (i - 1)) / 2 + (j - i)] = (uint16_t)((i << 8) | j);
@@ -108,9 +107,6 @@
     float* baug = reinterpret_cast<float*>(wslot + 16384);
     for (int e = tid; e < 512; e += SS_THREADS) baug[e] = 0.f;
   }
-  if (blockIdx.x == 0)
-    for (int e = tid; e < 2 * nkeys * SS_D; e += SS_THREADS)
-      a.centers[e] = __ldg(a.cen + (size_t)(e >> 6) * SS_D + (e & 31));
   if (tid == 0) {
     for (int b = 0; b < SS_NTB; ++b) {
       tc::mbar_init(&d1full[b], 1);
@@ -134,6 +130,13 @@
     tc::mbar_init(wempty, 1);
     tc::fence_barrier_init();
   }
+  if (warp == 4) tc::tmem_alloc(tmem_slot, SS_TMEM_COLS);
+  pdl_wait();
+  pdl_launch_dependents();
+  for (int j = tid; j <= nkeys; j += SS_THREADS) B[j] = __ldg(a.seg_off + j);
+  if (blockIdx.x == 0)
+    for (int e = tid; e < 2 * nkeys * SS_D; e += SS_THREADS)
+      a.centers[e] = __ldg(a.cen + (size_t)(e >> 6) * SS_D + (e & 31));
   __syncthreads();
   for (int r = tid; r < SS_TILE; r += SS_THREADS) {
     float* p = aaug + (r >> 3) * 64 + (r & 7) * 4;
@@ -155,7 +158,6 @@
       carry += __shfl_sync(0xffffffffu, v, 31);
     }
   }
-  if (warp == 4) tc::tmem_alloc(tmem_slot, SS_TMEM_COLS);
   tc::fence_proxy_async();
   tc::tc_fence_before();
   __syncthreads();
diff --git a/dpmmsubclusters.jl_b200/sweep.py b/dpmmsubclusters.jl_b200/sweep.py
--- a/dpmmsubclusters.jl_b200/sweep.py
+++ b/dpmmsubclusters.jl_b200/sweep.py
@@ -281,6 +281,12 @@
         self._ck(self.lib.dpmm_debug_tc_stats(self.h, _ptr(out, C.c_int64)))
         return (int(out[0]), int(out[1]), int(out[2])) if overflow else (int(out[0]), int(out[1]))
 
+    def sort_state(self):
+        perm = np.empty(self.n, np.int32)
+        moved = np.zeros(1, np.int64)
+        self._ck(self.lib.dpmm_debug_sort(self.h, _ptr(perm, C.c_int32), _ptr(moved, C.c_int64)))
+        return perm, int(moved[0])
+
     def fused_stats(self):
         out = np.zeros(3, np.int64)
         self._ck(self.lib.dpmm_debug_fused_stats(self.h, _ptr(out, C.c_int64)))
diff --git a/include/dpmm_b200.h b/include/dpmm_b200.h
--- a/include/dpmm_b200.h
+++ b/include/dpmm_b200.h
@@ -90,6 +90,7 @@
 int dpmm_set_uniforms(dpmm_ctx* ctx, const double* u_label, const double* u_sub, const uint8_t* r_bits);
 int dpmm_debug_loglik(dpmm_ctx* ctx, int32_t which, float* out);
 int dpmm_debug_tc_stats(dpmm_ctx* ctx, int64_t* out3);
+int dpmm_debug_sort(dpmm_ctx* ctx, int32_t* perm, int64_t* moved);
 int dpmm_debug_fused_stats(dpmm_ctx* ctx, int64_t* out3);
 int dpmm_timing_enable(dpmm_ctx* ctx, int32_t on);
 int dpmm_timing_kinds(void);
```

Result: faster. 5678 (median of 6 runs) (+5.9%).
